# HengyiWang/spann3r

Measured on AMD Instinct MI355X. Metric: frames/sec/GPU (224px, 10-frame seq) + mem-bank cross-attn HBM GB/s, higher is better.
Workload: dtype bf16; 1 GPU; Spann3R.forward, 10-frame 224x224 sequence, batch 1, ViT-L enc / ViT-B dec / DPT heads, eval memory policy; parallelism=sequences sharded 1/GPU x1, hip_graphs=True

## Files before the change

include/spann3r_hip.h:

```cpp
#ifndef SPANN3R_HIP_H
#define SPANN3R_HIP_H

#include <stdint.h>

#ifdef __cplusplus
extern "C" {
#endif

enum { SP3_F32 = 0, SP3_BF16 = 1 };
enum { SP3_ATTN_F32X3 = 2, SP3_ATTN_F16X3 = 3 };
enum { SP3_ACT_NONE = 0, SP3_ACT_GELU = 1, SP3_ACT_RELU = 2 };
enum { SP3_EPI_PLAIN = 0, SP3_EPI_ROPE_VT = 1, SP3_EPI_PIXSHUF = 2, SP3_EPI_PARTIAL = 3 };
enum { SP3_LOAD_PLAIN = 0, SP3_LOAD_CONV3X3 = 1, SP3_LOAD_SOFTMAX = 2 };

const char* sp3_last_error(void);
int sp3_version(void);

int sp3_weight_stream_set(int mode);
int sp3_weight_stream_get(void);

typedef struct sp3_gemm_desc {
  const float* A;
  const float* A2;
  const void* W;
// ... 75 lines not shown
  const float* g2; const float* b2; void* out2; int64_t ld2; int32_t out2_bf16;
  float eps;
  int32_t splits, rows, C;
  int32_t out1_packed, out2_packed;
  int32_t act;
  const float* res2;
  int64_t ldres2;
} sp3_reduce_ln_desc;
int sp3_reduce_ln(const sp3_reduce_ln_desc* desc_host, void* stream);

int sp3_rope_2d(void* tokens, int dtype, int B, int N, int H, int D, int64_t sB, int64_t sN, int64_t sH,
                const int64_t* positions, float base, float fwd, void* stream);

int sp3_attention(const void* q, int64_t sq, int64_t ldq, const void* k, int64_t sk, int64_t ldk,
                  const void* vt, int64_t vt_ld, void* out, int64_t ldo, int out_bf16,
                  int B, int heads, int Nq, int Nk, float scale, int dtype, void* stream);
int sp3_attention_ex(const void* q, int64_t sq, int64_t ldq, const void* k, int64_t sk, int64_t ldk,
                     const void* vt, int64_t vt_ld, void* out, int64_t ldo, int out_bf16, int out_packed,
                     int B, int heads, int Nq, int Nk, float scale, int dtype, void* stream);

int sp3_attention_packed(const void* qp, int q_cols, int q_col0, int npad_q, const void* kp, int k_cols, int k_col0, int npad_k,
                         const void* vtp, void* out, int64_t ldo, int out_bf16, int out_packed,
                         int B, int heads, int Nq, int Nk, float scale, int o_group, int o_group_rows, void* stream);

typedef struct sp3_attn_qproj_desc {
  const void* x_packed; int64_t x_group_stride;
  const float* ln_stats; int64_t stats_group_stride;
  const void* w_packed; int64_t w_group_stride;
  const float* ln_s; const float* bias; int64_t vec_group_stride;
  const int32_t* pos; const float* rope_cos; const float* rope_sin;
  float ln_eps; int32_t D;
  const void* kp; int32_t k_cols, k_col0, npad_k; const void* vtp;
  void* out; int64_t ldo; int32_t out_bf16, out_packed;
  int32_t B, heads, Nq, Nk; float scale; int32_t o_group, o_group_rows;
} sp3_attn_qproj_desc;
int sp3_attention_packed_qproj(const sp3_attn_qproj_desc* desc_host, void* stream);

typedef struct sp3_bank_write_desc {
  const float* feat_k;
  const float* feat_v;
  float* k_raw;
  float* v_raw;
  void* k_hat;
  void* v_hat_t;
  float* s_bank;
  float* b_bank;
  const float *gamma_k, *beta_k, *gamma_v, *beta_v, *gamma_q, *beta_q;
  float eps;
  float alpha;
  int32_t M, P, C, cap;
  int32_t wdtype;
  const int32_t* state;
} sp3_bank_write_desc;
int sp3_bank_write(const sp3_bank_write_desc* desc_host, void* stream);
int sp3_softmax_thresh(const float* S, float* P, int64_t ld, int64_t strideS, int rows, int M, int Mpad,
                       float thresh, int batch, void* P_packed, int64_t stride_packed, int packed_bf16, void* stream);
int sp3_softmax_pack(const float* S, int64_t ld, int64_t strideS, int rows, int M, float thresh, int batch, void* P_packed,
                     int64_t stride_packed, int packed_bf16, float* rowstat_ws, void* stream);
int sp3_colsum_accum(const float* P, int64_t ld, int rows, int M, float* mem_attn, void* stream);
int sp3_colsum_packed(const void* P_packed, int packed_bf16, int rows, int M, float* mem_attn, void* stream);
int sp3_colsum_softmax(const float* S, int64_t ld, int rows, int M, const float* rowz, float thresh, float* mem_attn,
                       float* mem_count, int append_P, void* stream);
int sp3_pack_stats(const float* x, int64_t ldx, int rows, int C, void* packed, int packed_bf16, float* stats, void* stream);
int sp3_gather_packed_rows(const void* src, void* dst, const int32_t* sel, int n_sel, int C, int elem_size, void* stream);
int sp3_gather_packed_cols(const void* src, void* dst, const int32_t* sel, int n_sel, int n_fill, int C, int cap,
                           int elem_size, void* stream);
int sp3_cos_sim(const float* k, const float* wm, int T, int P, int C, float* scratch, float* score, void* stream);
int sp3_bank_state_set(int32_t* state, int M, int wm, void* stream);
int sp3_prob_merge(const float* stats, float* scale, int rows, int M, int cap, const int32_t* dyn_n, void* stream);
int sp3_colsum_prob(const void* P_packed, const float* scale, int rows, int M, int cap, const int32_t* dyn_n, float* mem_attn, void* stream);
int sp3_cos_sim_state(const float* k, const float* k_raw, int Tmax, int P, int C, const int32_t* state, float* scratch, float* score,
                      void* stream);
int sp3_mem_append(float* count, float* attn, int M, int P, void* stream);
int sp3_prune_select(const float* attn, const float* count, int M, float protect, int top_k,
                     int32_t* sel, void* stream);
int sp3_gather_rows(const void* src, void* dst, const int32_t* sel, int n_sel, int C, int elem_size, void* stream);
int sp3_gather_cols(const void* src, int64_t ld_src, void* dst, int64_t ld_dst, const int32_t* sel, int n_sel,
                    int n_fill, int C, int elem_size, void* stream);
int sp3_gather_1d(const float* src, float* dst, const int32_t* sel, int n_sel, void* stream);

int sp3_conv3x3_tile(const void* x, int in_bf16, const void* w_packed, const float* bias, const float* res1,
                     const float* res2, void* out, int out_bf16, int res_bf16, int tile_px, int B, int H, int W,
                     int Cin, int Cout, int relu_in, int act, void* stream);
int sp3_im2col_patch(const float* img, int64_t sb, int64_t sc, int64_t sy, int64_t sx, int B, int C, int H, int W,
                     int p, void* out, int out_bf16, int out_packed, void* stream);
int sp3_upsample2x(const float* in, float* out, int B, int H, int W, int C, int outH, int outW, void* stream);
int sp3_upsample2x_bf16(const void* in, void* out, int B, int H, int W, int C, int outH, int outW, void* stream);
int sp3_head_final(const float* feat, const float* w, const float* b, int64_t pixels, int C, float* pts,
                   float* conf, float* raw, void* stream);
int sp3_head_final_bf16(const void* feat, const float* w, const float* b, int64_t pixels, int C, float* pts, float* conf,
                        float* raw, void* stream);

int sp3_preprocess_image(const uint8_t* src, int64_t src_row_stride, int crop_l, int crop_t, int H1, int W1,
                         const int32_t* hbounds, const int32_t* hcoef, int hksize, int W2,
                         const int32_t* vbounds, const int32_t* vcoef, int vksize, int H2,
                         int crop2_l, int crop2_t, int outW, int outH, int transpose, uint8_t* tmp, float* out, void* stream);

int64_t sp3_conf_loss_ws_bytes(int n, int B);
int sp3_conf_loss_forward(const float* P, const float* Cf, const float* G, const uint8_t* V, const float* pose0, int n, int B, int HW,
                          float alpha, int fix_first, void* ws, float* out7, float* ent_out, void* stream);
int sp3_conf_loss_backward(const float* P, const float* Cf, const float* G, const uint8_t* V, const float* pose0, int n, int B, int HW,
                           float alpha, int fix_first, const void* ws, const float* grad_scale2, float* dP, float* dC, void* stream);
int64_t sp3_ssi_loss_ws_bytes(int n, int B, int HW);
int sp3_ssi_loss_forward(const float* P, const float* G, const uint8_t* V, const float* pose0, int n, int B, int HW, int fix_first,
                         int gt_scale, void* ws, float* out, void* stream);
int sp3_ssi_align_stats(const float* P, const float* G, const uint8_t* V, const float* pose0, int n, int B, int HW, void* ws, float* stats,
                        void* stream);

int sp3_transpose(const float* src, int64_t ld_src, float* dst, int64_t ld_dst, int rows, int cols, void* stream);
int sp3_transpose_batched(const float* src, int64_t ld_src, int64_t stride_src, float* dst, int64_t ld_dst, int64_t stride_dst, int rows,
                          int cols, int batch, void* stream);
int sp3_transpose_pad(const float* src, int64_t ld_src, int64_t stride_src, float* dst, int64_t ld_dst, int64_t stride_dst, int rows,
                      int cols, int batch, int pad_to, void* stream);
int sp3_gelu(const float* x, float* y, int64_t n, void* stream);
int sp3_gelu_bwd(const float* x, const float* dy, float* dx, int64_t n, void* stream);
int sp3_im2col3x3(const float* x, float* col, int B, int H, int W, int C, int stride, void* stream);
int sp3_col2im3x3(const float* dcol, float* dx, int B, int H, int W, int C, int stride, void* stream);
int sp3_relu(const float* x, float* y, int64_t n, void* stream);
int sp3_relu_bwd(const float* x, const float* dy, float* dx, int64_t n, void* stream);
int sp3_upsample2x_bwd(const float* dy, float* dx, int B, int H, int W, int C, int outH, int outW, void* stream);
int sp3_postprocess(const float* raw, float* pts, float* conf, int64_t M, void* stream);
int sp3_postprocess_bwd(const float* raw, const float* dpts, const float* dconf, float* draw, int64_t M, void* stream);
int sp3_adamw(float* p, const float* g, float* m, float* v, int64_t n, float lr, float beta1, float beta2, float eps, float weight_decay,
              int step, float grad_scale, void* stream);
int sp3_mul(const float* a, const float* b, float* out, int64_t n, void* stream);
int sp3_pack_bf16(const float* src, int64_t ld, int rows, int cols, void* dst, void* dstT, void* stream);
int sp3_pack_bf16_conv3x3(const float* x, int B, int H, int W, int C, int stride, int act, void* dst, void* dstT, void* stream);
int sp3_pack_bf16_act(const float* src, int64_t ld, int rows, int cols, void* dst, void* dstT, int act, void* stream);
int sp3_pack_bf16_colsum(const float* src, int64_t ld, int rows, int cols, void* dst, void* dstT, float* colsum, int accumulate,
                         float* partial_ws, void* stream);
int64_t sp3_sumsq_blocks(int64_t n);
int64_t sp3_colsum_rows_ws(int rows, int N);
int sp3_colsum_rows(const float* x, int64_t ld, int rows, int N, float* out, int accumulate, float* scratch, void* stream);
int sp3_sumsq_partial(const float* g, int64_t n, double* partial, void* stream);
int sp3_clip_coef(const double* partial, int count, float max_norm, float extra_scale, float* out, int* step_counter, void* stream);
int sp3_adamw_flat(float* p, const float* g, float* m, float* v, int64_t n, const float* chunk_table, float lr, float beta1, float beta2,
                   float eps, int step, const float* grad_scale_dev, float grad_scale, const int* step_dev, const float* lr_dev, void* stream);
int sp3_softmax_bwd(const float* A, const float* dAd, const float* mask, float* dS, int64_t ld, int rows, int T, float alpha, void* stream);
int sp3_softmax_bwd_pad(const float* A, const float* dAd, const float* mask, float* dS, int64_t ld, int rows, int T, int Tpad, float alpha,
                        void* stream);
typedef struct sp3_head_part {
  const float* src;
  int64_t s_b, s_n, s_h;
  float* dst;
  int64_t d_b, d_n, d_h;
  float* dstT;
  const int64_t* pos;
  int32_t N;
  float fwd;
  int64_t ldT;
} sp3_head_part;
int sp3_head_shuffle(const sp3_head_part* parts, int nparts, int B, int H, int hd, float rope_base, const float* cos_tab,
                     const float* sin_tab, int tab_len, void* stream);
int sp3_attention_train_fwd(const float* q, int64_t sq, int64_t ldq, const float* k, int64_t sk, int64_t ldk, const float* vt, int64_t vt_ld,
                            float* out, int64_t ldo, float* lse, int B, int heads, int Nq, int Nk, float scale, int bf16_products, void* stream);
typedef struct sp3_attn_bwd_desc {
  const float *q, *k, *v, *dout;
  int64_t sq, ldq, sk, ldk, sv, ldv, sdo, lddo;
  const float *qT, *kT, *doT;
  int64_t ldTq, ldTk;
  const float* lse;
  float* D;
  float *dq, *dk, *dv;
  int64_t sdq, lddq, sdk, lddk, sdv, lddv;
  int32_t B, heads, Nq, Nk;
  float scale;
  int32_t bf16_products;
} sp3_attn_bwd_desc;
int sp3_attention_train_bwd(const sp3_attn_bwd_desc* d, void* stream);
int sp3_layernorm_bwd(const float* x, int64_t ldx, const float* gamma, const float* dy, int64_t ldy, const float* dx_add, int64_t ld_add,
                      float* dx, int64_t ld_dx, float* dgamma, float* dbeta, int accumulate, float* scratch, int rows, int C, float eps,
                      void* stream);

int sp3_focal_weiszfeld(const float* pts3d, int B, int H, int W, float ppx, float ppy, int iters, float focal_min, float focal_max,
// ... 184 lines not shown
```

spann3r_amd/csrc/conv.hip:

```cpp
#include "common.h"
#include <type_traits>
#include <cstdlib>

namespace {

constexpr int TH = 8, TW = 8;
constexpr int HP = (TH + 2) * (TW + 2);
constexpr int BM = TH * TW, BN = 64;
constexpr int MF = BM / 16, NF = BN / 16;
constexpr int SLAB_LD = BN + 4;
constexpr int DEPTH = 3;
constexpr int SP3_CONV_WIDE_MIN_WGS = 256;

struct ConvArgs {
  const void* x; const __bf16* w; const float* bias; const float* res1; const float* res2; void* out;
  int B, H, W, Cin, Cout, tiles_x, tiles_y, relu_in, act, out_bf16;
  int xcd_nb;
};

__device__ __forceinline__ bool conv_tile_of(const ConvArgs& a, int& t, int& nblk) {
  t = blockIdx.x; nblk = blockIdx.y;
  if (a.xcd_nb) {
    const unsigned L = blockIdx.x, xc = L & 7, jj = L >> 3, q = jj / (unsigned)a.xcd_nb;
    nblk = (int)(jj - q * a.xcd_nb);
    t = (int)(q * 8 + xc);
    if (t >= a.tiles_x * a.tiles_y * a.B) return false;
  }
  return true;
}

__device__ __forceinline__ bf16x8 ld_frag_lds(const char* p) { return *reinterpret_cast<const bf16x8*>(p); }

template <typename TIN>
__global__ __launch_bounds__(256) void conv3x3_tile_kernel(const ConvArgs a) {
  extern __shared__ __attribute__((aligned(16))) char lds[];
  const int tid = threadIdx.x, lane = tid & 63, wave = tid >> 6, g = lane >> 4, r = lane & 15;
  const int Cin = a.Cin;
  const int PS = Cin * 2 + 16;
  int t, nblk;
  if (!conv_tile_of(a, t, nblk)) return;
  const int tx = t % a.tiles_x; t /= a.tiles_x;
  const int ty = t % a.tiles_y;
  const int b = t / a.tiles_y;
  const int y0 = ty * TH, x0 = tx * TW, n0 = nblk * BN;

  const int upt = Cin >> 5;
  const int U = 9 * upt;
  const int nkb = (9 * Cin) >> 6;
  const __bf16* wb[NF];
#pragma unroll
  for (int n = 0; n < NF; ++n) wb[n] = a.w + ((int64_t)((n0 >> 4) + n) * nkb * 128 + lane) * 8;
  const int nu = (U - wave + 3) >> 2;
  auto w_off = [&](int i) -> int64_t {
    int u = wave + 4 * i;
    u = u < U ? u : U - 1;
    return (int64_t)(u >> 1) * (64 * 16) + (u & 1) * (64 * 8);
  };
  bf16x8 wq[DEPTH][NF];
#pragma unroll
  for (int s = 0; s < DEPTH; ++s) {
    const int64_t o = w_off(s);
#pragma unroll
    for (int n = 0; n < NF; ++n) wq[s][n] = *reinterpret_cast<const bf16x8*>(wb[n] + o);
  }

  {
    constexpr int CHK = 16 / (int)sizeof(TIN);
    const int cpp = Cin / CHK;
    const TIN* xin = reinterpret_cast<const TIN*>(a.x) + (int64_t)b * a.H * a.W * Cin;
    using Chunk = typename std::conditional<sizeof(TIN) == 4, float4, bf16x8>::type;
    auto src_of = [&](int p, int c, bool& ok) -> const Chunk* {
      const int hy = p / (TW + 2), hx = p - hy * (TW + 2);
      const int iy = y0 + hy - 1, ix = x0 + hx - 1;
      ok = p < HP && iy >= 0 && iy < a.H && ix >= 0 && ix < a.W;
      const int cy = ok ? iy : 0, cx = ok ? ix : 0;
      return reinterpret_cast<const Chunk*>(xin + ((int64_t)cy * a.W + cx) * Cin + c);
    };
    auto put = [&](int p, int c, Chunk v, bool ok) {
      char* dst = lds + p * PS + c * 2;
      if constexpr (sizeof(TIN) == 4) {
        if (!ok) v = make_float4(0.f, 0.f, 0.f, 0.f);
        if (a.relu_in) v = relu4(v);
        bf16x4 o;
        o[0] = (__bf16)v.x; o[1] = (__bf16)v.y; o[2] = (__bf16)v.z; o[3] = (__bf16)v.w;
        *reinterpret_cast<bf16x4*>(dst) = o;
      } else {
#pragma unroll
        for (int e = 0; e < 8; ++e) {
          const float f = (float)v[e];
          v[e] = (ok && (!a.relu_in || f > 0.f)) ? v[e] : (__bf16)0.f;
        }
        *reinterpret_cast<bf16x8*>(dst) = v;
      }
    };
    if ((256 % cpp) == 0) {
      const int c = (tid % cpp) * CHK, pstep = 256 / cpp;
      constexpr int NB = 13;
      for (int p0 = tid / cpp; p0 < HP; p0 += NB * pstep) {
        Chunk buf[NB];
        bool ok[NB];
// ... 33 lines not shown
    return (ky * (TW + 2) + kx) * PS + (((c32 >> 1) << 6) + 16 * g + ((c32 & 1) << 3)) * 2;
  };
  bf16x8 af[2][MF];
  {
    const int o = a_off(0);
#pragma unroll
    for (int m = 0; m < MF; ++m) af[0][m] = ld_frag_lds(lds + abase[m] + o);
  }
  for (int i0 = 0; i0 < nu; i0 += 2 * DEPTH) {
#pragma unroll
    for (int s2 = 0; s2 < 2 * DEPTH; ++s2) {
      const int i = i0 + s2;
      if (i < nu) {
        const int s = s2 % DEPTH, cur = s2 & 1;
        {
          const int o = a_off(i + 1);
#pragma unroll
          for (int m = 0; m < MF; ++m) af[cur ^ 1][m] = ld_frag_lds(lds + abase[m] + o);
        }
#pragma unroll
        for (int m = 0; m < MF; ++m)
#pragma unroll
          for (int n = 0; n < NF; ++n)
            acc[m][n] = __builtin_amdgcn_mfma_f32_16x16x32_bf16(af[cur][m], wq[s][n], acc[m][n], 0, 0, 0);
        {
          const int64_t o = w_off(i + DEPTH);
#pragma unroll
          for (int n = 0; n < NF; ++n) wq[s][n] = *reinterpret_cast<const bf16x8*>(wb[n] + o);
        }
      }
    }
  }
  __syncthreads();

  float* slab = reinterpret_cast<float*>(lds) + (size_t)wave * BM * SLAB_LD;
#pragma unroll
  for (int m = 0; m < MF; ++m)
#pragma unroll
    for (int n = 0; n < NF; ++n)
#pragma unroll
      for (int q = 0; q < 4; ++q) slab[(m * 16 + 4 * g + q) * SLAB_LD + n * 16 + r] = acc[m][n][q];
  __syncthreads();
  const float* sm = reinterpret_cast<const float*>(lds);
  for (int idx = tid; idx < BM * (BN / 4); idx += 256) {
    const int row = idx / (BN / 4), c4 = (idx % (BN / 4)) * 4;
    const int oy = y0 + row / TW, ox = x0 + row % TW;
    if (oy >= a.H || ox >= a.W) continue;
    float4 v = *reinterpret_cast<const float4*>(sm + row * SLAB_LD + c4);
#pragma unroll
    for (int s = 1; s < 4; ++s) {
      const float4 t4 = *reinterpret_cast<const float4*>(sm + (size_t)s * BM * SLAB_LD + row * SLAB_LD + c4);
      v.x += t4.x; v.y += t4.y; v.z += t4.z; v.w += t4.w;
    }
    const int gn = n0 + c4;
    if (a.bias) { const float4 b4 = *reinterpret_cast<const float4*>(a.bias + gn); v.x += b4.x; v.y += b4.y; v.z += b4.z; v.w += b4.w; }
    if (a.act == SP3_ACT_RELU) v = relu4(v);
    const int64_t off = (((int64_t)b * a.H + oy) * a.W + ox) * a.Cout + gn;
    if (a.out_bf16 & 2) {
      if (a.res1) { const bf16x4 q = *reinterpret_cast<const bf16x4*>(reinterpret_cast<const __bf16*>(a.res1) + off); v.x += (float)q[0]; v.y += (float)q[1]; v.z += (float)q[2]; v.w += (float)q[3]; }
      if (a.res2) { const bf16x4 q = *reinterpret_cast<const bf16x4*>(reinterpret_cast<const __bf16*>(a.res2) + off); v.x += (float)q[0]; v.y += (float)q[1]; v.z += (float)q[2]; v.w += (float)q[3]; }
    } else {
      if (a.res1) { const float4 q = *reinterpret_cast<const float4*>(a.res1 + off); v.x += q.x; v.y += q.y; v.z += q.z; v.w += q.w; }
      if (a.res2) { const float4 q = *reinterpret_cast<const float4*>(a.res2 + off); v.x += q.x; v.y += q.y; v.z += q.z; v.w += q.w; }
    }
    if (a.out_bf16 & 1) {
      bf16x4 o;
      o[0] = (__bf16)v.x; o[1] = (__bf16)v.y; o[2] = (__bf16)v.z; o[3] = (__bf16)v.w;
      st_out(reinterpret_cast<bf16x4*>(reinterpret_cast<__bf16*>(a.out) + off), o);
    } else {
      st_out(reinterpret_cast<float4*>(reinterpret_cast<float*>(a.out) + off), v);
    }
  }
}

namespace wide {
constexpr int TH = 8, TW = 16, HW = TW + 2, HP = (TH + 2) * HW;
constexpr int CH = 128, PS = CH * 2 + 16;
constexpr int MF = 8;
constexpr int HALO_BYTES = HP * PS;
template <int NF> constexpr int lds_bytes() {
  return HALO_BYTES > 4 * 64 * (16 * NF + 4) * 4 ? HALO_BYTES : 4 * 64 * (16 * NF + 4) * 4;
}

template <typename TIN, int NF = 4, int ABL = 0, bool WS = false>
__global__ __launch_bounds__(256, 2) void conv3x3_wide_kernel(const ConvArgs a) {
  constexpr int BN = 16 * NF, SLAB_LD = BN + 4;
  constexpr int DEPTH = NF == 2 ? 9 : 3;
  static_assert(9 % DEPTH == 0, "the queue slot of a tap must not depend on the chunk");
  extern __shared__ __attribute__((aligned(16))) char lds[];
  const int tid = threadIdx.x, lane = tid & 63, wave = tid >> 6, g = lane >> 4, r = lane & 15;
  const int Cin = a.Cin;
  int t, nblk;
  if (!conv_tile_of(a, t, nblk)) return;
  const int tx = t % a.tiles_x; t /= a.tiles_x;
  const int ty = t % a.tiles_y;
  const int b = t / a.tiles_y;
  const int y0 = ty * TH, x0 = tx * TW, n0 = nblk * BN;
  const int nchunk = Cin / CH, upt = Cin >> 5;
  const int total = 9 * nchunk;

  typedef __attribute__((ext_vector_type(4))) uint32_t u32x4;
  const int nkb = (9 * Cin) >> 6;
  const uint32_t panel_bytes = (uint32_t)nkb * 128 * 8 * 2;
  const auto wrsrc = __builtin_amdgcn_make_buffer_rsrc(
      const_cast<char*>(reinterpret_cast<const char*>(a.w)) + (int64_t)(n0 >> 4) * panel_bytes, 0, (int)(NF * panel_bytes), 0x00020000);
  const uint32_t wlane = (uint32_t)lane * 16 + (uint32_t)(wave & 1) * 1024;
  const int wave_u = __builtin_amdgcn_readfirstlane(wave);
  auto w_off = [&](int c, int tap) -> uint32_t {
    return (uint32_t)((tap * upt + 4 * c + wave_u) >> 1) * 2048;
  };
  auto w_off_seq = [&](int seq) -> uint32_t {
    seq = seq < total ? seq : total - 1;
    const int c = seq / 9;
    return w_off(c, seq - 9 * c);
  };
  auto w_load = [&](uint32_t o, bf16x8* dst) {
#pragma unroll
    for (int n = 0; n < NF; ++n) {
      const u32x4 v = __builtin_amdgcn_raw_buffer_load_b128(wrsrc, wlane, o + n * panel_bytes, WS ? SP3_AUX_STREAM : SP3_AUX_DEFAULT);
      dst[n] = *reinterpret_cast<const bf16x8*>(&v);
    }
  };
  bf16x8 wq[DEPTH][NF];
#pragma unroll
  for (int s = 0; s < DEPTH; ++s) w_load(DEPTH == 9 ? w_off(0, s) : w_off_seq(s), wq[s]);

  f32x4 acc[MF][NF];
#pragma unroll
  for (int m = 0; m < MF; ++m)
#pragma unroll
    for (int n = 0; n < NF; ++n) acc[m][n] = f32x4{0.f, 0.f, 0.f, 0.f};
  const char* abase = lds + r * PS + (((wave >> 1) << 6) + 16 * g + ((wave & 1) << 3)) * 2;

  constexpr int CHK = 16 / (int)sizeof(TIN);
  constexpr int CPP = CH / CHK;
  constexpr int PSTEP = 256 / CPP, NB = sizeof(TIN) == 4 ? 6 : 12;
  const uint32_t img_bytes = (uint32_t)(a.H * a.W * Cin) * (uint32_t)sizeof(TIN);
  const auto rsrc = __builtin_amdgcn_make_buffer_rsrc(
      const_cast<char*>(reinterpret_cast<const char*>(a.x)) + (int64_t)b * img_bytes, 0, (int)img_bytes, 0x00020000);
  const uint32_t xlane = (uint32_t)((tid % CPP) * CHK * sizeof(TIN));
  char* hdst = lds + (tid % CPP) * CHK * 2;

  u32x4 buf[NB];
  auto issue = [&](int c, int p0) {
#pragma unroll
    for (int q = 0; q < NB; ++q) {
      const int p = p0 + q * PSTEP;
      const int hy = p / HW, hx = p - hy * HW;
      const int iy = y0 + hy - 1, ix = x0 + hx - 1;
      const bool ok = p < HP && iy >= 0 && iy < a.H && ix >= 0 && ix < a.W;
      const uint32_t off = ok ? (uint32_t)((iy * a.W + ix) * Cin + c * CH) * (uint32_t)sizeof(TIN) + xlane : 0x80000000u;
      if constexpr (ABL & 4) buf[q] = u32x4{0u, 0u, 0u, 0u};
      else buf[q] = __builtin_amdgcn_raw_buffer_load_b128(rsrc, off, 0, 0);
    }
  };
  auto commit = [&](int p0) {
#pragma unroll
    for (int q = 0; q < NB; ++q) {
      const int p = p0 + q * PSTEP;
      if (p >= HP) continue;
      char* dst = hdst + p * PS;
      if constexpr (sizeof(TIN) == 4) {
        float4 v = make_float4(__uint_as_float(buf[q][0]), __uint_as_float(buf[q][1]), __uint_as_float(buf[q][2]), __uint_as_float(buf[q][3]));
        if (a.relu_in) v = relu4(v);
        bf16x4 o;
        o[0] = (__bf16)v.x; o[1] = (__bf16)v.y; o[2] = (__bf16)v.z; o[3] = (__bf16)v.w;
        *reinterpret_cast<bf16x4*>(dst) = o;
      } else {
        u32x4 v = buf[q];
        if (a.relu_in) {
#pragma unroll
          for (int e = 0; e < 4; ++e) {
            const uint32_t neg = v[e] & 0x80008000u;
            v[e] &= ~((neg >> 15) * 0xffffu);
          }
        }
        *reinterpret_cast<u32x4*>(dst) = v;
      }
    }
  };
  for (int c = 0; c < nchunk; ++c) {
    if (c) __syncthreads();
    for (int p0 = tid / CPP; p0 < HP; p0 += NB * PSTEP) {
      issue(c, p0);
      commit(p0);
    }
    __syncthreads();

    bf16x8 af[MF];
#pragma unroll
    for (int m = 0; m < MF; ++m) af[m] = ld_frag_lds(abase + m * HW * PS);
#pragma unroll
    for (int tap = 0; tap < 9; ++tap) {
      const int s = tap % DEPTH;
      const int nt = tap + 1, nky = nt / 3, nkx = nt - 3 * nky;
#pragma unroll
      for (int m = 0; m < MF; ++m) {
#pragma unroll
        for (int n = 0; n < NF; ++n)
          acc[m][n] = __builtin_amdgcn_mfma_f32_16x16x32_bf16(af[m], wq[s][n], acc[m][n], 0, 0, 0);
        if constexpr (!(ABL & 2))
          if (tap < 8) af[m] = ld_frag_lds(abase + ((m + nky) * HW + nkx) * PS);
      }
      if constexpr (!(ABL & 1)) {
        if constexpr (DEPTH == 9) { if (c + 1 < nchunk) w_load(w_off(c + 1, tap), wq[s]); }
        else w_load(w_off_seq(9 * c + tap + DEPTH), wq[s]);
      }
    }
  }

  float* slab = reinterpret_cast<float*>(lds) + (size_t)wave * 64 * SLAB_LD;
  const float* sm = reinterpret_cast<const float*>(lds);
  if constexpr (ABL & 8) {
    float sum = 0.f;
#pragma unroll
    for (int m = 0; m < MF; ++m)
#pragma unroll
      for (int n = 0; n < NF; ++n) sum += acc[m][n][0] + acc[m][n][1] + acc[m][n][2] + acc[m][n][3];
    if (sum == 12345.678f) reinterpret_cast<float*>(a.out)[tid] = sum;
    return;
  }
#pragma unroll
  for (int h = 0; h < 2; ++h) {
    __syncthreads();
#pragma unroll
    for (int m = 0; m < 4; ++m)
#pragma unroll
      for (int n = 0; n < NF; ++n)
#pragma unroll
        for (int q = 0; q < 4; ++q) slab[(m * 16 + 4 * g + q) * SLAB_LD + n * 16 + r] = acc[4 * h + m][n][q];
    __syncthreads();
    for (int idx = tid; idx < 64 * (BN / 4); idx += 256) {
      const int row = idx / (BN / 4), c4 = (idx % (BN / 4)) * 4;
      const int oy = y0 + 4 * h + (row >> 4), ox = x0 + (row & 15);
      if (oy >= a.H || ox >= a.W) continue;
      float4 v = *reinterpret_cast<const float4*>(sm + row * SLAB_LD + c4);
#pragma unroll
      for (int s = 1; s < 4; ++s) {
        const float4 t4 = *reinterpret_cast<const float4*>(sm + (size_t)s * 64 * SLAB_LD + row * SLAB_LD + c4);
        v.x += t4.x; v.y += t4.y; v.z += t4.z; v.w += t4.w;
      }
      const int gn = n0 + c4;
      if (a.bias) { const float4 b4 = *reinterpret_cast<const float4*>(a.bias + gn); v.x += b4.x; v.y += b4.y; v.z += b4.z; v.w += b4.w; }
      if (a.act == SP3_ACT_RELU) v = relu4(v);
      const int64_t off = (((int64_t)b * a.H + oy) * a.W + ox) * a.Cout + gn;
      if (a.out_bf16 & 2) {
        if (a.res1) { const bf16x4 q = *reinterpret_cast<const bf16x4*>(reinterpret_cast<const __bf16*>(a.res1) + off); v.x += (float)q[0]; v.y += (float)q[1]; v.z += (float)q[2]; v.w += (float)q[3]; }
        if (a.res2) { const bf16x4 q = *reinterpret_cast<const bf16x4*>(reinterpret_cast<const __bf16*>(a.res2) + off); v.x += (float)q[0]; v.y += (float)q[1]; v.z += (float)q[2]; v.w += (float)q[3]; }
      } else {
        if (a.res1) { const float4 q = *reinterpret_cast<const float4*>(a.res1 + off); v.x += q.x; v.y += q.y; v.z += q.z; v.w += q.w; }
        if (a.res2) { const float4 q = *reinterpret_cast<const float4*>(a.res2 + off); v.x += q.x; v.y += q.y; v.z += q.z; v.w += q.w; }
      }
      if (a.out_bf16 & 1) {
        bf16x4 o;
        o[0] = (__bf16)v.x; o[1] = (__bf16)v.y; o[2] = (__bf16)v.z; o[3] = (__bf16)v.w;
        st_out(reinterpret_cast<bf16x4*>(reinterpret_cast<__bf16*>(a.out) + off), o);
      } else {
        st_out(reinterpret_cast<float4*>(reinterpret_cast<float*>(a.out) + off), v);
      }
    }
  }
}

template <typename TIN, int NF, bool WS>
int launch(dim3 grid, hipStream_t st, const ConvArgs& a) {
  constexpr int lds = lds_bytes<NF>();
  auto kern = conv3x3_wide_kernel<TIN, NF, 0, WS>;
  if (lds > 64 * 1024) {
    static bool raised = false;
    if (!raised) {
      hipError_t e = hipFuncSetAttribute(reinterpret_cast<const void*>(kern), hipFuncAttributeMaxDynamicSharedMemorySize, lds);
      if (e != hipSuccess) { sp3_set_error("sp3_conv3x3_tile: cannot raise dynamic LDS to %d: %s", lds, hipGetErrorString(e)); return 2; }
      raised = true;
    }
  }
  hipLaunchKernelGGL(kern, grid, dim3(256), lds, st, a);
  return 0;
}
}

}

extern "C" int sp3_conv3x3_tile(const void* x, int in_bf16, const void* w_packed, const float* bias, const float* res1,
                                const float* res2, void* out, int out_bf16, int res_bf16, int tile_px, int B, int H, int W,
                                int Cin, int Cout, int relu_in, int act, void* stream) {
  SP3_CHECK(x && w_packed && out, "sp3_conv3x3_tile: null pointer");
  SP3_CHECK(B > 0 && H > 0 && W > 0, "sp3_conv3x3_tile: bad shape");
  SP3_CHECK(Cin % 64 == 0 && Cin >= 64 && Cout % 64 == 0 && Cout >= 64, "sp3_conv3x3_tile: Cin=%d / Cout=%d must be multiples of 64", Cin, Cout);
  SP3_CHECK(act == SP3_ACT_NONE || act == SP3_ACT_RELU, "sp3_conv3x3_tile: act %d", act);
  SP3_CHECK(out_bf16 == 0 || out_bf16 == 1, "sp3_conv3x3_tile: out_bf16 %d is not 0 or 1", out_bf16);
  SP3_CHECK(res_bf16 == 0 || res_bf16 == 1, "sp3_conv3x3_tile: res_bf16 %d is not 0 or 1", res_bf16);
  SP3_CHECK(tile_px >= 0 && tile_px <= 3, "sp3_conv3x3_tile: tile_px %d is not 0..3", tile_px);
  auto al16 = [](const void* q) { return (reinterpret_cast<uintptr_t>(q) & 15) == 0; };
  SP3_CHECK(al16(x) && al16(w_packed) && al16(bias) && al16(res1) && al16(res2) && al16(out), "sp3_conv3x3_tile: 16-byte alignment");
  ConvArgs a;
  a.x = x; a.w = reinterpret_cast<const __bf16*>(w_packed); a.bias = bias; a.res1 = res1; a.res2 = res2; a.out = out;
  a.B = B; a.H = H; a.W = W; a.Cin = Cin; a.Cout = Cout;
  a.relu_in = relu_in; a.act = act; a.out_bf16 = out_bf16 | (res_bf16 << 1);
  a.xcd_nb = 0;
  constexpr bool xcd_on = true;
  hipStream_t st = reinterpret_cast<hipStream_t>(stream);
  {
    const int want = tile_px;
    const int wtx = (W + wide::TW - 1) / wide::TW, wty = (H + wide::TH - 1) / wide::TH;
    const int64_t wgs = (int64_t)wtx * wty * B * (Cout / 64);
    const bool can = Cin % wide::CH == 0;
    SP3_CHECK(want < 2 || can, "sp3_conv3x3_tile: the 8 x 16 tile needs Cin %% 128 == 0 (Cin=%d)", Cin);
    SP3_CHECK((int64_t)H * W * Cin * (in_bf16 ? 2 : 4) < (1ll << 31), "sp3_conv3x3_tile: one image of the map must stay below 2 GiB");
    const int nf = want == 2 ? 4 : want == 3 ? 2 : (want == 0 && can) ? (wgs >= SP3_CONV_WIDE_MIN_WGS ? 4 : wgs >= 80 ? 2 : 0) : 0;
    if (nf) {
      a.tiles_x = wtx; a.tiles_y = wty;
      dim3 grid(wtx * wty * B, Cout / (16 * nf));
      if (xcd_on) { a.xcd_nb = Cout / (16 * nf); grid = dim3((unsigned)(((wtx * wty * B + 7) / 8) * 8 * a.xcd_nb), 1); }
      const bool ws = sp3_weight_streams(SP3_WF_CONV_WIDE, nf);
      int rc;
      if (nf == 4) rc = in_bf16 ? (ws ? wide::launch<__bf16, 4, true>(grid, st, a) : wide::launch<__bf16, 4, false>(grid, st, a))
                                : (ws ? wide::launch<float, 4, true>(grid, st, a) : wide::launch<float, 4, false>(grid, st, a));
      else         rc = in_bf16 ? (ws ? wide::launch<__bf16, 2, true>(grid, st, a) : wide::launch<__bf16, 2, false>(grid, st, a))
                                : (ws ? wide::launch<float, 2, true>(grid, st, a) : wide::launch<float, 2, false>(grid, st, a));
      if (rc) return rc;
      SP3_LAUNCH_CHECK("sp3_conv3x3_tile");
      return 0;
    }
  }
  a.tiles_x = (W + TW - 1) / TW; a.tiles_y = (H + TH - 1) / TH;
  const size_t halo = (size_t)HP * (Cin * 2 + 16), slabs = (size_t)4 * BM * SLAB_LD * sizeof(float);
  const size_t lds = halo > slabs ? halo : slabs;
  SP3_CHECK(lds <= 160 * 1024, "sp3_conv3x3_tile: Cin=%d needs %zu bytes of LDS", Cin, lds);
  dim3 grid(a.tiles_x * a.tiles_y * B, Cout / BN);
  if (xcd_on) { a.xcd_nb = Cout / BN; grid = dim3((unsigned)(((a.tiles_x * a.tiles_y * B + 7) / 8) * 8 * a.xcd_nb), 1); }
  auto launch = [&](auto kern) -> int {
    static size_t raised = 0;
    if (lds > 64 * 1024 && lds > raised) {
      raised = lds;
      hipError_t e = hipFuncSetAttribute(reinterpret_cast<const void*>(kern), hipFuncAttributeMaxDynamicSharedMemorySize, (int)lds);
      if (e != hipSuccess) { sp3_set_error("sp3_conv3x3_tile: cannot raise dynamic LDS to %zu: %s", lds, hipGetErrorString(e)); return 2; }
    }
    hipLaunchKernelGGL(kern, grid, dim3(256), lds, st, a);
    return 0;
  };
  const int rc = in_bf16 ? launch(conv3x3_tile_kernel<__bf16>) : launch(conv3x3_tile_kernel<float>);
  if (rc) return rc;
  SP3_LAUNCH_CHECK("sp3_conv3x3_tile");
  return 0;
}
```

spann3r_amd/csrc/dpt.hip:

```cpp
#include "common.h"
#include <math.h>

namespace {

__global__ __launch_bounds__(256) void im2col_patch_kernel(const float* __restrict__ img, int64_t sb, int64_t sc, int64_t sy,
                                                           int64_t sx, int C, int H, int W, int p, void* __restrict__ out,
                                                           int out_bf16, int out_packed, int64_t total) {
  const int64_t idx = (int64_t)blockIdx.x * 256 + threadIdx.x;
  if (idx >= total) return;
  const int K = C * p * p;
  const int64_t row = idx / K;
  const int k = (int)(idx - row * K);
  const int nw = W / p, nh = H / p;
  const int b = (int)(row / (nh * nw));
  const int rem = (int)(row - (int64_t)b * nh * nw);
  const int ty = rem / nw, tx = rem - ty * nw;
  const int c = k / (p * p), r2 = k - c * p * p;
  const int iy = r2 / p, ix = r2 - iy * p;
  const float val = img[b * sb + c * sc + (int64_t)(ty * p + iy) * sy + (int64_t)(tx * p + ix) * sx];
  const int64_t o = out_packed ? packed_off((int)row, k, K, out_bf16 != 0) : idx;
  if (out_bf16) reinterpret_cast<__bf16*>(out)[o] = (__bf16)val;
  else reinterpret_cast<float*>(out)[o] = val;
}

__device__ __forceinline__ float4 ld4(const float* p) { return *reinterpret_cast<const float4*>(p); }
__device__ __forceinline__ float4 ld4(const __bf16* p) {
  const bf16x4 t = *reinterpret_cast<const bf16x4*>(p);
  return make_float4((float)t[0], (float)t[1], (float)t[2], (float)t[3]);
}
__device__ __forceinline__ void st4(float* p, const float4 v) { st_out(reinterpret_cast<float4*>(p), v); }
__device__ __forceinline__ void st4(__bf16* p, const float4 v) {
  bf16x4 t;
  t[0] = (__bf16)v.x; t[1] = (__bf16)v.y; t[2] = (__bf16)v.z; t[3] = (__bf16)v.w;
  st_out(reinterpret_cast<bf16x4*>(p), t);
}

template <typename T>
__global__ __launch_bounds__(256) void upsample2x_kernel(const T* __restrict__ in, T* __restrict__ out, int H, int W,
                                                         int C, int outH, int outW, int64_t total4) {
  const int64_t idx = (int64_t)blockIdx.x * 256 + threadIdx.x;
  if (idx >= total4) return;
  const int c4 = C >> 2;
  const int cc = (int)(idx % c4);
  int64_t pix = idx / c4;
  const int ox = (int)(pix % outW);
  pix /= outW;
  const int oy = (int)(pix % outH);
  const int b = (int)(pix / outH);
  const int OH = 2 * H, OW = 2 * W;
  const float sh = OH > 1 ? (float)(H - 1) / (float)(OH - 1) : 0.f;
  const float sw = OW > 1 ? (float)(W - 1) / (float)(OW - 1) : 0.f;
  const float fy = sh * (float)oy, fx = sw * (float)ox;
  int y0 = (int)fy, x0 = (int)fx;
  y0 = y0 < H - 1 ? y0 : H - 1;
  x0 = x0 < W - 1 ? x0 : W - 1;
  const int y1 = y0 < H - 1 ? y0 + 1 : y0, x1 = x0 < W - 1 ? x0 + 1 : x0;
  const float ly = fy - (float)y0, lx = fx - (float)x0;
  const float hy = 1.f - ly, hx = 1.f - lx;
  const T* base = in + (int64_t)b * H * W * C;
  const float4 v00 = ld4(base + (((int64_t)y0 * W + x0) * c4 + cc) * 4);
  const float4 v01 = ld4(base + (((int64_t)y0 * W + x1) * c4 + cc) * 4);
  const float4 v10 = ld4(base + (((int64_t)y1 * W + x0) * c4 + cc) * 4);
  const float4 v11 = ld4(base + (((int64_t)y1 * W + x1) * c4 + cc) * 4);
  float4 o;
  o.x = hy * (hx * v00.x + lx * v01.x) + ly * (hx * v10.x + lx * v11.x);
  o.y = hy * (hx * v00.y + lx * v01.y) + ly * (hx * v10.y + lx * v11.y);
  o.z = hy * (hx * v00.z + lx * v01.z) + ly * (hx * v10.z + lx * v11.z);
  o.w = hy * (hx * v00.w + lx * v01.w) + ly * (hx * v10.w + lx * v11.w);
  st4(out + idx * 4, o);
}

__global__ __launch_bounds__(256) void upsample2x_bf16x8_kernel(const __bf16* __restrict__ in, __bf16* __restrict__ out, int H, int W,
                                                                int C, int outH, int outW) {
  const int c8 = C >> 3;
  const int t = blockIdx.x * 256 + threadIdx.x;
  if (t >= outW * c8) return;
  const int ox = t / c8, cg = t - ox * c8;
  const int oy = blockIdx.y, b = blockIdx.z;
  const int OH = 2 * H, OW = 2 * W;
  const float sh = OH > 1 ? (float)(H - 1) / (float)(OH - 1) : 0.f;
  const float sw = OW > 1 ? (float)(W - 1) / (float)(OW - 1) : 0.f;
  const float fy = sh * (float)oy, fx = sw * (float)ox;
  int y0 = (int)fy, x0 = (int)fx;
  y0 = y0 < H - 1 ? y0 : H - 1;
  x0 = x0 < W - 1 ? x0 : W - 1;
  const int y1 = y0 < H - 1 ? y0 + 1 : y0, x1 = x0 < W - 1 ? x0 + 1 : x0;
  const float ly = fy - (float)y0, lx = fx - (float)x0;
  const float hy = 1.f - ly, hx = 1.f - lx;
  const __bf16* base = in + (int64_t)b * H * W * C + cg * 8;
  const bf16x8 v00 = *reinterpret_cast<const bf16x8*>(base + ((int64_t)y0 * W + x0) * C);
  const bf16x8 v01 = *reinterpret_cast<const bf16x8*>(base + ((int64_t)y0 * W + x1) * C);
  const bf16x8 v10 = *reinterpret_cast<const bf16x8*>(base + ((int64_t)y1 * W + x0) * C);
  const bf16x8 v11 = *reinterpret_cast<const bf16x8*>(base + ((int64_t)y1 * W + x1) * C);
  bf16x8 o;
#pragma unroll
  for (int e = 0; e < 8; ++e)
    o[e] = (__bf16)(hy * (hx * (float)v00[e] + lx * (float)v01[e]) + ly * (hx * (float)v10[e] + lx * (float)v11[e]));
  st_out(reinterpret_cast<bf16x8*>(out + (((int64_t)b * outH + oy) * outW + ox) * C + cg * 8), o);
}

template <typename T>
__global__ __launch_bounds__(256) void head_final_kernel(const T* __restrict__ feat, const float* __restrict__ w,
                                                         const float* __restrict__ bias, int64_t pixels, int C,
                                                         float* __restrict__ pts, float* __restrict__ conf,
                                                         float* __restrict__ raw) {
  const int64_t gid = (int64_t)blockIdx.x * 256 + threadIdx.x;
  const int64_t pix = gid >> 3;
  const int sub = (int)(gid & 7);
  const bool valid = pix < pixels;
  const int64_t pp = valid ? pix : pixels - 1;
  float a0 = 0.f, a1 = 0.f, a2 = 0.f, a3 = 0.f;
  const T* f = feat + pp * C;
  for (int c = sub * 4; c < C; c += 32) {
    const float4 x = ld4(f + c);
    const float4 w0 = *reinterpret_cast<const float4*>(w + c);
    const float4 w1 = *reinterpret_cast<const float4*>(w + C + c);
    const float4 w2 = *reinterpret_cast<const float4*>(w + 2 * C + c);
    const float4 w3 = *reinterpret_cast<const float4*>(w + 3 * C + c);
    a0 += (x.x * w0.x + x.y * w0.y) + (x.z * w0.z + x.w * w0.w);
    a1 += (x.x * w1.x + x.y * w1.y) + (x.z * w1.z + x.w * w1.w);
    a2 += (x.x * w2.x + x.y * w2.y) + (x.z * w2.z + x.w * w2.w);
    a3 += (x.x * w3.x + x.y * w3.y) + (x.z * w3.z + x.w * w3.w);
  }
#pragma unroll
  for (int o = 1; o < 8; o <<= 1) {
    a0 += __shfl_xor(a0, o); a1 += __shfl_xor(a1, o); a2 += __shfl_xor(a2, o); a3 += __shfl_xor(a3, o);
  }
  if (valid && sub == 0) {
    const float x = a0 + bias[0], y = a1 + bias[1], z = a2 + bias[2], c = a3 + bias[3];
    if (raw) { raw[pix * 4 + 0] = x; raw[pix * 4 + 1] = y; raw[pix * 4 + 2] = z; raw[pix * 4 + 3] = c; }
    const float d = sqrtf(x * x + y * y + z * z);
    const float sc = expm1f(d) / fmaxf(d, 1e-8f);
    pts[pix * 3 + 0] = x * sc; pts[pix * 3 + 1] = y * sc; pts[pix * 3 + 2] = z * sc;
    conf[pix] = 1.0f + expf(c);
  }
}

template <int LP, int PPT>
__global__ __launch_bounds__(256) void head_final_bf16x8_kernel(const __bf16* __restrict__ feat, const float* __restrict__ w,
                                                                const float* __restrict__ bias, int64_t pixels, float* __restrict__ pts,
                                                                float* __restrict__ conf, float* __restrict__ raw) {
  constexpr int C = 8 * LP, PPB = 256 / LP;
  const int li = threadIdx.x % LP, pl = threadIdx.x / LP;
  float wr[4][8];
#pragma unroll
  for (int f = 0; f < 4; ++f) {
    const float4 a = *reinterpret_cast<const float4*>(w + f * C + li * 8), b = *reinterpret_cast<const float4*>(w + f * C + li * 8 + 4);
    wr[f][0] = a.x; wr[f][1] = a.y; wr[f][2] = a.z; wr[f][3] = a.w; wr[f][4] = b.x; wr[f][5] = b.y; wr[f][6] = b.z; wr[f][7] = b.w;
  }
  const float b0 = bias[0], b1 = bias[1], b2 = bias[2], b3 = bias[3];
  const int64_t p0 = (int64_t)blockIdx.x * PPB * PPT + pl;
  bf16x8 x[PPT];
#pragma unroll
  for (int q = 0; q < PPT; ++q) {
    int64_t pix = p0 + (int64_t)q * PPB;
    pix = pix < pixels ? pix : pixels - 1;
    x[q] = *reinterpret_cast<const bf16x8*>(feat + pix * C + li * 8);
  }
#pragma unroll
  for (int q = 0; q < PPT; ++q) {
    const int64_t pix = p0 + (int64_t)q * PPB;
    float a[4];
#pragma unroll
    for (int f = 0; f < 4; ++f) {
      float t0 = 0.f, t1 = 0.f;
#pragma unroll
      for (int e = 0; e < 4; ++e) { t0 = fmaf((float)x[q][e], wr[f][e], t0); t1 = fmaf((float)x[q][4 + e], wr[f][4 + e], t1); }
      a[f] = t0 + t1;
    }
#pragma unroll
    for (int o = 1; o < LP; o <<= 1) {
      a[0] += __shfl_xor(a[0], o); a[1] += __shfl_xor(a[1], o); a[2] += __shfl_xor(a[2], o); a[3] += __shfl_xor(a[3], o);
    }
    if (li == 0 && pix < pixels) {
      const float X = a[0] + b0, Y = a[1] + b1, Z = a[2] + b2, Cc = a[3] + b3;
      if (raw) *reinterpret_cast<float4*>(raw + pix * 4) = make_float4(X, Y, Z, Cc);
      const float d = sqrtf(X * X + Y * Y + Z * Z);
      const float sc = expm1f(d) / fmaxf(d, 1e-8f);
      pts[pix * 3 + 0] = X * sc; pts[pix * 3 + 1] = Y * sc; pts[pix * 3 + 2] = Z * sc;
      conf[pix] = 1.0f + expf(Cc);
    }
  }
}

}

#define ST(s) reinterpret_cast<hipStream_t>(s)

extern "C" int sp3_im2col_patch(const float* img, int64_t sb, int64_t sc, int64_t sy, int64_t sx, int B, int C, int H, int W,
                                int p, void* out, int out_bf16, int out_packed, void* stream) {
  SP3_CHECK(img && out && B > 0 && C > 0 && p > 0, "sp3_im2col_patch: bad arguments");
  SP3_CHECK(H % p == 0 && W % p == 0, "Input image size (%d,%d) is not a multiple of patch size (%d)", H, W, p);
  const int64_t total = (int64_t)B * (H / p) * (W / p) * C * p * p;
  hipLaunchKernelGGL(im2col_patch_kernel, dim3((unsigned)((total + 255) / 256)), dim3(256), 0, ST(stream), img, sb, sc, sy, sx,
                     C, H, W, p, out, out_bf16, out_packed, total);
  SP3_LAUNCH_CHECK("sp3_im2col_patch");
  return 0;
}

extern "C" int sp3_upsample2x(const float* in, float* out, int B, int H, int W, int C, int outH, int outW, void* stream) {
  SP3_CHECK(in && out && B > 0 && H > 0 && W > 0 && C > 0 && C % 4 == 0, "sp3_upsample2x: bad arguments");
  SP3_CHECK(outH > 0 && outH <= 2 * H && outW > 0 && outW <= 2 * W, "sp3_upsample2x: bad crop");
  const int64_t total4 = (int64_t)B * outH * outW * (C / 4);
  hipLaunchKernelGGL(upsample2x_kernel<float>, dim3((unsigned)((total4 + 255) / 256)), dim3(256), 0, ST(stream), in, out, H, W, C,
                     outH, outW, total4);
  SP3_LAUNCH_CHECK("sp3_upsample2x");
  return 0;
}

extern "C" int sp3_upsample2x_bf16(const void* in, void* out, int B, int H, int W, int C, int outH, int outW, void* stream) {
  SP3_CHECK(in && out && B > 0 && H > 0 && W > 0 && C > 0 && C % 4 == 0, "sp3_upsample2x_bf16: bad arguments");
  SP3_CHECK(outH > 0 && outH <= 2 * H && outW > 0 && outW <= 2 * W, "sp3_upsample2x_bf16: bad crop");
  if (C % 8 == 0 && outH <= 65535 && B <= 65535) {
    hipLaunchKernelGGL(upsample2x_bf16x8_kernel, dim3((unsigned)((outW * (C / 8) + 255) / 256), outH, B), dim3(256), 0, ST(stream),
                       reinterpret_cast<const __bf16*>(in), reinterpret_cast<__bf16*>(out), H, W, C, outH, outW);
    SP3_LAUNCH_CHECK("sp3_upsample2x_bf16");
    return 0;
  }
  const int64_t total4 = (int64_t)B * outH * outW * (C / 4);
  hipLaunchKernelGGL(upsample2x_kernel<__bf16>, dim3((unsigned)((total4 + 255) / 256)), dim3(256), 0, ST(stream),
                     reinterpret_cast<const __bf16*>(in), reinterpret_cast<__bf16*>(out), H, W, C, outH, outW, total4);
  SP3_LAUNCH_CHECK("sp3_upsample2x_bf16");
  return 0;
}

extern "C" int sp3_head_final(const float* feat, const float* w, const float* b, int64_t pixels, int C, float* pts, float* conf,
                              float* raw, void* stream) {
  SP3_CHECK(feat && w && b && pts && conf && pixels > 0 && C > 0 && C % 32 == 0, "sp3_head_final: bad arguments");
  const int64_t threads = pixels * 8;
  hipLaunchKernelGGL(head_final_kernel<float>, dim3((unsigned)((threads + 255) / 256)), dim3(256), 0, ST(stream), feat, w, b, pixels, C,
                     pts, conf, raw);
  SP3_LAUNCH_CHECK("sp3_head_final");
  return 0;
}

extern "C" int sp3_head_final_bf16(const void* feat, const float* w, const float* b, int64_t pixels, int C, float* pts, float* conf,
                                   float* raw, void* stream) {
  SP3_CHECK(feat && w && b && pts && conf && pixels > 0 && C > 0 && C % 32 == 0, "sp3_head_final_bf16: bad arguments");
  if (C == 128 && (reinterpret_cast<uintptr_t>(feat) & 15) == 0 && (reinterpret_cast<uintptr_t>(w) & 15) == 0 && (!raw || (reinterpret_cast<uintptr_t>(raw) & 15) == 0)) {
    constexpr int LP = 16, PPT = 4, PPB = 256 / LP;
    hipLaunchKernelGGL((head_final_bf16x8_kernel<LP, PPT>), dim3((unsigned)((pixels + PPB * PPT - 1) / (PPB * PPT))), dim3(256), 0, ST(stream),
                       reinterpret_cast<const __bf16*>(feat), w, b, pixels, pts, conf, raw);
    SP3_LAUNCH_CHECK("sp3_head_final_bf16");
    return 0;
  }
  const int64_t threads = pixels * 8;
  hipLaunchKernelGGL(head_final_kernel<__bf16>, dim3((unsigned)((threads + 255) / 256)), dim3(256), 0, ST(stream),
                     reinterpret_cast<const __bf16*>(feat), w, b, pixels, C, pts, conf, raw);
  SP3_LAUNCH_CHECK("sp3_head_final_bf16");
  return 0;
}
```

spann3r_amd/engine.py:

```python
import math
import os

import torch

from . import ops
from .lib import ACT_NONE, ACT_GELU, ACT_RELU
from .config import Spann3RConfig


def _rope_tables(max_pos, base, device):
    half = 32
    inv_freq = 1.0 / (base ** (torch.arange(0, half, 2).float() / half))
    t = torch.arange(max_pos, dtype=torch.float32)
    ang = torch.einsum("i,j->ij", t, inv_freq)
    return ang.cos().contiguous().to(device), ang.sin().contiguous().to(device)


def _rope_tables_narrow(max_pos, base, head_dim, device):
    D = head_dim // 2
    nf = D // 2
    assert nf <= 16 and head_dim % 4 == 0
    inv_freq = 1.0 / (base ** (torch.arange(0, D, 2).float() / D))
    t = torch.arange(max_pos, dtype=torch.float32)
    ang = torch.einsum("i,j->ij", t, inv_freq)
# ... 480 lines not shown
                                 ln=ops.LnFold(stq, D, w[g + "cq.s"], 1e-6, sb_stats=sb_st, sb_s=D * 4),
                                 strideA=xq.stride, strideW=w[g + "cq.w"].stride, strideC=B * npad * D, sb={"bias": D * 4}, **rope)
                ops.attention_packed(cqp, D, 0, npad, ckp, D, 0, npad, cvtp, ao, D, B=2 * B, heads=Hh, Nq=P, Nk=P,
                                     scale=64 ** -0.5, o_group=B, o_group_rows=Rp)
            upd(ao, D, "cproj", xo, stq, xq)
            Hd = D * cfg.mlp_ratio
            ops.gemm(xq, w[g + "fc1.w"], h, M=R, N=Hd, K=D, lda=D, ldc=Hd, bias=w[g + "fc1.b"], act=ACT_GELU,
                     ln=ops.LnFold(stq, D, w[g + "fc1.s"], 1e-6, sb_stats=sb_st, sb_s=Hd * 4),
                     batch=2, strideA=xq.stride, strideW=w[g + "fc1.w"].stride, strideC=h.stride, sb={"bias": Hd * 4})
            if last:
                upd(h, Hd, "fc2", xo, None, None)
            else:
                upd(h, Hd, "fc2", xo, st[nx], xp[nx])
        normed = self.ws("decg_normed", (2, R, D))
        ops.layernorm(x[depth], w["dec_norm.w"], w["dec_norm.b"], 1e-6, normed, rows=2 * R, C_=D,
                      dual=self.wspg("decg_normed_packed", R, D) if self.adt == torch.bfloat16 else None, group_rows=R)
        outs = {}
        for s_ in (0, 1):
            outs[s_] = [(f1, f2)[s_]] + [x[l][s_].view(B, P, D) for l in range(1, depth)] + [normed[s_].view(B, P, D)]
        return outs[0], outs[1]

    def key_aux(self, R):
        E = self.cfg.enc_dim
        return self.wspg("keyg_packed", R, E), self.ws("keyg_stats", (2, R, E // 32, 2))

    def encode_feat_keys_grouped(self, feat1, feat2, normed1, normed2, R, out1, out2, feat1p=None, feat2p=None, aux=None):
        self.activate()
        cfg, w = self.cfg, self.w
        E, D, Kd = cfg.enc_dim, cfg.dec_dim, cfg.key_dim
        dF, dN, dO = feat2.data_ptr() - feat1.data_ptr(), normed2.data_ptr() - normed1.data_ptr(), out2.data_ptr() - out1.data_ptr()
        assert dF % 16 == 0 and dN % 16 == 0 and dO % 16 == 0
        es = 2 if self.adt == torch.bfloat16 else 4
        h = self.wspg("keyg_hidden", R, Kd)
        packed = None
        if feat1p is not None and feat2p is not None and self.adt == torch.bfloat16 and ops.LEAN:
            np_ = self.wspg("decg_normed_packed", R, D)
            dFp = feat2p.data_ptr() - feat1p.data_ptr()
            assert dFp % 16 == 0
            packed = dict(A2=np_, lda2=D, K1=E, batch=2, strideA=dFp // 2, strideW=w["keyg.0.w"].stride, strideC=h.stride,
                          sb={"bias": Kd * 4, "A2": np_.stride * 2})
            ok = self._splitA_plan.get(R)
            if ok is None:
                ok = self._splitA_plan[R] = ops.gemm(feat1p, w["keyg.0.w"], h, M=R, N=Kd, K=Kd, lda=E, ldc=Kd, bias=w["keyg.0.b"],
                                                     act=ACT_GELU, plan_only=True, **packed) >= 30
            if not ok:
                packed = None
        if packed is not None:
            ops.gemm(feat1p, w["keyg.0.w"], h, M=R, N=Kd, K=Kd, lda=E, ldc=Kd, bias=w["keyg.0.b"], act=ACT_GELU, **packed)
        else:
            ops.gemm(feat1, w["keyg.0.w"], h, M=R, N=Kd, K=Kd, lda=E, ldc=Kd, bias=w["keyg.0.b"], act=ACT_GELU, A2=normed1, lda2=D, K1=E,
                     batch=2, strideA=dF // 4, strideW=w["keyg.0.w"].stride, strideC=h.stride, sb={"bias": Kd * 4, "A2": dN})
        kp, kst = aux or self.key_aux(R)
        ops.gemm(h, w["keyg.2.w"], out1, M=R, N=E, K=Kd, lda=Kd, ldc=E, bias=w["keyg.2.b"], stats_out=kst, c2=kp,
                 batch=2, strideA=h.stride, strideW=w["keyg.2.w"].stride, strideC=dO // 4,
                 sb={"bias": E * 4, "stats_out": R * (E // 32) * 8, "c2": kp.stride * es})
        return kp.at(1), kst[1]

    def encode_feat_key(self, feat, dec_last, R, num, out, aux=False):
        self.activate()
        cfg, w = self.cfg, self.w
        E, D, Kd = cfg.enc_dim, cfg.dec_dim, cfg.key_dim
        h = self.wsp("key_hidden%d" % num, R, Kd)
        pre = "key%d." % num
        ops.gemm(feat, w[pre + "0.w"], h, M=R, N=Kd, K=Kd, lda=E, ldc=Kd, bias=w[pre + "0.b"], act=ACT_GELU,
                 A2=dec_last, lda2=D, K1=E)
        if aux:
            kp, kst = self.key_aux(R) if aux is True else aux
            ops.gemm(h, w[pre + "2.w"], out, M=R, N=E, K=Kd, lda=Kd, ldc=E, bias=w[pre + "2.b"], stats_out=kst[num - 1],
                     c2=kp.at(num - 1))
            return kp.at(num - 1), kst[num - 1]
        ops.gemm(h, w[pre + "2.w"], out, M=R, N=E, K=Kd, lda=Kd, ldc=E, bias=w[pre + "2.b"])
        return out

    def _conv_ws(self, head):
        return self.ws("conv_splitk_ws" + str(head), (1 << 23,))

    def _rcu_c1(self, x, pre, B, H, W_, tag=""):
        w, F = self.w, self.cfg.dpt_feat
        t = self.ws("rcu_tmp" + tag, (B * H * W_, F), self.mdt)
        ops.conv3x3(x, w[pre + "c1.w"], t, B=B, H=H, W_=W_, Cin=F, Cout=F, bias=w[pre + "c1.b"], relu_in=True, act=ACT_RELU,
                    splitk_ws=self._conv_ws(tag[:1]))
        return t

    def _rcu(self, x, pre, B, H, W_, out, extra_res=None, tag="", c1_done=False, extra_up=None):
        w, F = self.w, self.cfg.dpt_feat
        t = self.ws("rcu_tmp" + tag, (B * H * W_, F), self.mdt)
        if not c1_done:
            self._rcu_c1(x, pre, B, H, W_, tag)
        ops.conv3x3(t, w[pre + "c2.w"], out, B=B, H=H, W_=W_, Cin=F, Cout=F, bias=w[pre + "c2.b"], res1=x, res2=extra_res,
                    splitk_ws=self._conv_ws(tag[:1]), res2_up=extra_up)
        return out

    def _fusion(self, pre, B, H, W_, x0, x1, tag, crop=None, c1_done=False, x0_up=None, fold_up=False):
        w, F = self.w, self.cfg.dpt_feat
        M = B * H * W_
        cur = x0
        if x1 is not None:
            s = self.ws("fus_sum_" + tag, (M, F), self.mdt)
            self._rcu(x1, pre + "u1", B, H, W_, s, extra_res=x0, tag=tag, c1_done=c1_done, extra_up=x0_up)
            cur = s
        r = self.ws("fus_rcu2_" + tag, (M, F), self.mdt)
        self._rcu(cur, pre + "u2", B, H, W_, r, tag=tag, c1_done=c1_done and x1 is None)
        oc = self.ws("fus_oc_" + tag, (M, F), self.mdt)
        ops.gemm(r, w[pre + "out.w"], oc, M=M, N=F, K=F, lda=F, ldc=F, bias=w[pre + "out.b"])
        OH, OW = (2 * H, 2 * W_) if crop is None else crop
        if fold_up:
            return oc, OH, OW
        up = self.ws("fus_up_" + tag, (B * OH * OW, F), self.mdt)
        ops.upsample2x(oc, up, B=B, H=H, W_=W_, C_=F, outH=OH, outW=OW)
        return up, OH, OW

    def dpt_head(self, dec, B, nh, nw, num, want_raw=False):
        self.activate()
        cfg, w = self.cfg, self.w
        F, Lc = cfg.dpt_feat, cfg.dpt_last
        pre = "dpt%d." % num
        R = B * nh * nw
        hk = cfg.hooks
        dims = (cfg.enc_dim, cfg.dec_dim, cfg.dec_dim, cfg.dec_dim)
        ld = (96, 192, 384, 768)
        mdt = self.mdt
        t = [self.ws("dpt%d_pp%d" % (num, i), (R, ld[i]), mdt) for i in range(4)]
        import contextlib
        lv = ops.HEAD_LEVELS
        group = ops.level if len({dec[hk[i]].dtype for i in range(4)}) == 1 else contextlib.nullcontext
        with (group if lv else contextlib.nullcontext)():
            for i0 in (0, 2):
                with (contextlib.nullcontext if lv else group)():
                    for i in (i0, i0 + 1):
                        ops.gemm(dec[hk[i]], w[pre + "pp%d.w" % i], t[i], M=R, N=ld[i], K=dims[i], lda=dims[i], ldc=ld[i], bias=w[pre + "pp%d.b" % i])
        c0 = 128 if self.wdt == torch.bfloat16 else ld[0]
        l0 = self.ws("dpt%d_l0" % num, (B * 16 * nh * nw, c0), mdt)
        l1 = self.ws("dpt%d_l1" % num, (B * 4 * nh * nw, ld[1]), mdt)
        with group():
            ops.conv_transpose_ks(t[0], w[pre + "pp0t.w"], l0, B=B, H=nh, W_=nw, Cin=ld[0], Cout=c0, ks=4, bias=w[pre + "pp0t.b"])
            ops.conv_transpose_ks(t[1], w[pre + "pp1t.w"], l1, B=B, H=nh, W_=nw, Cin=ld[1], Cout=ld[1], ks=2, bias=w[pre + "pp1t.b"])
        l2 = t[2]
        h3, w3 = (nh - 1) // 2 + 1, (nw - 1) // 2 + 1
        l3 = self.ws("dpt%d_l3" % num, (B * h3 * w3, ld[3]), mdt)
        sk = self._conv_ws(num)
        geo = ((4 * nh, 4 * nw), (2 * nh, 2 * nw), (nh, nw), (h3, w3))
        srcs = (l0, l1, l2, l3)
        rn = [self.ws("dpt%d_rn%d" % (num, i), (B * geo[i][0] * geo[i][1], F), mdt) for i in range(4)]

        def layer_rn(i):
            ops.conv3x3(srcs[i], w[pre + "rn%d.w" % i], rn[i], B=B, H=geo[i][0], W_=geo[i][1], Cin=(c0 if i == 0 else ld[i]), Cout=F, splitk_ws=sk)

        def pp3c():
            ops.conv3x3(t[3], w[pre + "pp3c.w"], l3, B=B, H=nh, W_=nw, Cin=ld[3], Cout=ld[3], stride=2, bias=w[pre + "pp3c.b"], splitk_ws=sk)

        refs = [(pre + "ref%d." % (4 - j), "%d_%d" % (num, 4 - j)) for j in range(4)]
        if lv:
            with ops.level():
                pp3c()
                layer_rn(2)
            with ops.level():
                layer_rn(0)
                layer_rn(1)
                layer_rn(3)
                self._rcu_c1(rn[2], refs[1][0] + "u1", B, geo[2][0], geo[2][1], refs[1][1])
            with ops.level():
                self._rcu_c1(rn[3], refs[0][0] + "u2", B, geo[3][0], geo[3][1], refs[0][1])
                self._rcu_c1(rn[1], refs[2][0] + "u1", B, geo[1][0], geo[1][1], refs[2][1])
                self._rcu_c1(rn[0], refs[3][0] + "u1", B, geo[0][0], geo[0][1], refs[3][1])
        else:
            pp3c()
            for i in range(4):
                layer_rn(i)
        path, up, Hc, Wc = rn[3], None, h3, w3
        for j in range(4):
            Hn, Wn = geo[3 - j]
            fold = lv and j < 3 and ops.conv3x3_takes_res2_up(w[refs[j + 1][0] + "u1c2.w"], mdt, B, *geo[2 - j])
            nxt, OH_, OW_ = self._fusion(refs[j][0], B, Hn, Wn, path, rn[3 - j] if j else None, refs[j][1], crop=(nh, nw) if j == 0 else None,
                                         c1_done=lv, x0_up=up, fold_up=fold)
            path, up = nxt, ((Hn, Wn) if fold else None)
        p1, H1, W1 = path, OH_, OW_
        a = self.ws("dpt%d_h0" % num, (B * H1 * W1, Lc), mdt)
        ops.conv3x3(p1, w[pre + "h0.w"], a, B=B, H=H1, W_=W1, Cin=F, Cout=Lc, bias=w[pre + "h0.b"])
        OH, OW = 2 * H1, 2 * W1
        u = self.ws("dpt%d_h0up" % num, (B * OH * OW, Lc), mdt)
        ops.upsample2x(a, u, B=B, H=H1, W_=W1, C_=Lc)
        c = self.ws("dpt%d_h2" % num, (B * OH * OW, Lc), mdt)
        ops.conv3x3(u, w[pre + "h2.w"], c, B=B, H=OH, W_=OW, Cin=Lc, Cout=Lc, bias=w[pre + "h2.b"], act=ACT_RELU)
        pts = self.ws("dpt_pts%d" % num, (B, OH, OW, 3))
        conf = self.ws("dpt_conf%d" % num, (B, OH, OW))
        raw = self.ws("dpt_raw%d" % num, (B, OH, OW, 4)) if want_raw else None
        ops.head_final(c, w[pre + "h4.w"], w[pre + "h4.b"], B * OH * OW, Lc, pts, conf, raw)
        return pts, conf, raw

    def encode_cur_value_feat(self, tok, out, res, pos32=None):
        self.activate()
        cfg, w = self.cfg, self.w
        B, P, Cv = tok.shape
        assert Cv == cfg.val_dim
        R, E = B * P, cfg.enc_dim
        zero_pos = self.ws("valf_zero_pos", (R, 2), torch.int32, zero=True)
        rope_tab = None
        if cfg.mem_pos_enc:
            assert pos32 is not None and self.rope_narrow is not None
            zero_pos, rope_tab = pos32, self.rope_narrow
        x = self.ws("valf_x", (R, Cv))
        xpA, xpB = self.wsp("valf_xpA", R, Cv), self.wsp("valf_xpB", R, Cv)
        stA, stB = self.stats("valf_stA", R, Cv), self.stats("valf_stB", R, Cv)
        ops.copy2d(tok.reshape(R, Cv), Cv, x, Cv, R, Cv)
        ops.pack_stats(x, xpA, stA, rows=R, C_=Cv)
        for i in range(cfg.val_depth):
            self._block(x, xpA, stA, xpB, stB, R, B, P, Cv, cfg.enc_heads, "val%d." % i, zero_pos, tag="_valf",
                        head_dim=Cv // cfg.enc_heads, rope_tab=rope_tab)
        ops.gemm(xpA, w["value_out.w"], out, M=R, N=E, K=Cv, lda=Cv, ldc=E, bias=w["value_out.b"], res1=res, ldr1=E,
                 ln=ops.LnFold(stA, Cv, w["value_out.s"], 1e-6))
        return out

    def encode_cur_value(self, pts3d, out, res):
        self.activate()
        cfg, w = self.cfg, self.w
        B, H, W_, _ = pts3d.shape
        p, E = cfg.patch, cfg.enc_dim
        nh, nw = H // p, W_ // p
        P = nh * nw
        R = B * P
        _, pos32, zero_pos = self.positions(B, nh, nw)
        col = self.wsp("im2col_val", R, 3 * p * p)
        sb, sy, sx, sc = pts3d.stride()
        ops.im2col_patch(pts3d, col, B=B, C_=3, H=H, W_=W_, p=p, strides=(sb, sc, sy, sx))
        x, xp, st = self._vit(col, R, B, P, "pospatch", "val", cfg.val_depth, pos32 if cfg.mem_pos_enc else zero_pos, tag="_val")
        ops.gemm(xp, w["value_out.w"], out, M=R, N=E, K=E, lda=E, ldc=E, bias=w["value_out.b"], res1=res, ldr1=E,
                 ln=ops.LnFold(st, E, w["value_out.s"], 1e-6))
        return out
```

spann3r_amd/lib.py:

```python
import ctypes as C
import os

import torch

_HERE = os.path.dirname(os.path.abspath(__file__))
LIB_PATH = os.environ.get("SP3_LIB_PATH") or os.path.join(_HERE, "libspann3r_hip.so")

F32, BF16 = 0, 1
ATTN_F32X3, ATTN_F16X3 = 2, 3
ACT_NONE, ACT_GELU, ACT_RELU = 0, 1, 2
EPI_PLAIN, EPI_ROPE_VT, EPI_PIXSHUF, EPI_PARTIAL = 0, 1, 2, 3
LOAD_PLAIN, LOAD_CONV3X3, LOAD_SOFTMAX = 0, 1, 2


class GemmDesc(C.Structure):
    _fields_ = [
        ("A", C.c_void_p), ("A2", C.c_void_p), ("W", C.c_void_p), ("C", C.c_void_p), ("bias", C.c_void_p),
        ("res1", C.c_void_p), ("res2", C.c_void_p),
        ("M", C.c_int32), ("N", C.c_int32), ("K", C.c_int32), ("batch", C.c_int32),
        ("K1", C.c_int32),
        ("lda", C.c_int64), ("lda2", C.c_int64), ("ldw", C.c_int64), ("ldc", C.c_int64),
        ("ldr1", C.c_int64), ("ldr2", C.c_int64),
        ("strideA", C.c_int64), ("strideW", C.c_int64), ("strideC", C.c_int64),
        ("alpha", C.c_float), ("wdtype", C.c_int32), ("act", C.c_int32), ("out_bf16", C.c_int32),
# ... 73 lines not shown
    _fields_ = [("ox", C.c_float), ("oy", C.c_float), ("oz", C.c_float), ("h", C.c_float), ("inv_h", C.c_float), ("slack", C.c_float),
                ("nx", C.c_int32), ("ny", C.c_int32), ("nz", C.c_int32)]


class RenderCam(C.Structure):
    _fields_ = [("R", C.c_float * 9), ("t", C.c_float * 3), ("fx", C.c_float), ("fy", C.c_float), ("cx", C.c_float), ("cy", C.c_float),
                ("width", C.c_int32), ("height", C.c_int32), ("z_near", C.c_float), ("point_size", C.c_int32)]


class ViewDesc(C.Structure):
    _fields_ = [("src", C.c_void_p), ("row_stride", C.c_int64), ("dtype", C.c_int32), ("src_w", C.c_int32), ("src_h", C.c_int32),
                ("crop_l", C.c_int32), ("crop_t", C.c_int32), ("W1", C.c_int32), ("H1", C.c_int32), ("W2", C.c_int32), ("H2", C.c_int32),
                ("l2", C.c_int32), ("t2", C.c_int32), ("w", C.c_int32), ("h", C.c_int32), ("transpose", C.c_int32),
                ("fu", C.c_float), ("fv", C.c_float), ("cu", C.c_float), ("cv", C.c_float), ("pose", C.c_float * 12),
                ("use_raw_invalid", C.c_int32), ("raw_invalid", C.c_float), ("depth_div", C.c_float), ("min_depth", C.c_float),
                ("max_depth", C.c_float)]


class TsdfFrame(C.Structure):
    _fields_ = [("depth", C.c_void_p), ("pts", C.c_void_p), ("valid", C.c_void_p), ("pixel_weight", C.c_void_p), ("rgba", C.c_void_p),
                ("row_stride", C.c_int64), ("w", C.c_int32), ("h", C.c_int32), ("fu", C.c_float), ("fv", C.c_float), ("cu", C.c_float),
                ("cv", C.c_float), ("w2c", C.c_float * 12)]


class TsdfView(C.Structure):
    _fields_ = [("depth", C.c_void_p), ("vertex", C.c_void_p), ("normal", C.c_void_p), ("rgba", C.c_void_p), ("row_stride", C.c_int64),
                ("w", C.c_int32), ("h", C.c_int32), ("fu", C.c_float), ("fv", C.c_float), ("cu", C.c_float), ("cv", C.c_float),
                ("c2w", C.c_float * 12), ("near", C.c_float), ("far", C.c_float)]


_lib = None

_PROTOS = {
    "sp3_gemm": [C.POINTER(GemmDesc), C.c_void_p],
    "sp3_gemm_n": [C.POINTER(C.POINTER(GemmDesc)), C.c_int, C.c_void_p],
    "sp3_gemm_plan_n": [C.POINTER(C.POINTER(GemmDesc)), C.c_int, C.POINTER(C.c_int)],
    "sp3_gemm_plan": [C.POINTER(GemmDesc)],
    "sp3_layernorm": [C.c_void_p, C.c_int64, C.c_void_p, C.c_void_p, C.c_float, C.c_void_p, C.c_int64, C.c_int,
                      C.c_int, C.c_int, C.c_void_p],
    "sp3_reduce_ln": [C.POINTER(ReduceLnDesc), C.c_void_p],
    "sp3_layernorm_dual": [C.c_void_p, C.c_int64, C.c_void_p, C.c_void_p, C.c_float, C.c_void_p, C.c_int64, C.c_void_p, C.c_int, C.c_int,
                           C.c_int, C.c_int, C.c_void_p],
    "sp3_layernorm_packed": [C.c_void_p, C.c_int64, C.c_void_p, C.c_void_p, C.c_float, C.c_void_p, C.c_int,
                             C.c_int, C.c_int, C.c_void_p],
    "sp3_attention_ex": [C.c_void_p, C.c_int64, C.c_int64, C.c_void_p, C.c_int64, C.c_int64, C.c_void_p, C.c_int64,
                         C.c_void_p, C.c_int64, C.c_int, C.c_int, C.c_int, C.c_int, C.c_int, C.c_int, C.c_float, C.c_int,
                         C.c_void_p],
    "sp3_layernorm_t": [C.c_void_p, C.c_int64, C.c_void_p, C.c_void_p, C.c_float, C.c_void_p, C.c_int64, C.c_int,
                        C.c_int, C.c_int, C.c_void_p],
    "sp3_rope_2d": [C.c_void_p, C.c_int, C.c_int, C.c_int, C.c_int, C.c_int, C.c_int64, C.c_int64, C.c_int64,
                    C.c_void_p, C.c_float, C.c_float, C.c_void_p],
    "sp3_attention": [C.c_void_p, C.c_int64, C.c_int64, C.c_void_p, C.c_int64, C.c_int64, C.c_void_p, C.c_int64,
                      C.c_void_p, C.c_int64, C.c_int, C.c_int, C.c_int, C.c_int, C.c_int, C.c_float, C.c_int, C.c_void_p],
    "sp3_attention_packed": [C.c_void_p, C.c_int, C.c_int, C.c_int, C.c_void_p, C.c_int, C.c_int, C.c_int, C.c_void_p,
                             C.c_void_p, C.c_int64, C.c_int, C.c_int, C.c_int, C.c_int, C.c_int, C.c_int, C.c_float, C.c_int, C.c_int,
                             C.c_void_p],
    "sp3_attention_packed_qproj": [C.POINTER(AttnQProjDesc), C.c_void_p],
    "sp3_softmax_thresh": [C.c_void_p, C.c_void_p, C.c_int64, C.c_int64, C.c_int, C.c_int, C.c_int, C.c_float,
                           C.c_int, C.c_void_p, C.c_int64, C.c_int, C.c_void_p],
    "sp3_softmax_pack": [C.c_void_p, C.c_int64, C.c_int64, C.c_int, C.c_int, C.c_float, C.c_int, C.c_void_p, C.c_int64, C.c_int, C.c_void_p,
                         C.c_void_p],
    "sp3_colsum_packed": [C.c_void_p, C.c_int, C.c_int, C.c_int, C.c_void_p, C.c_void_p],
    "sp3_colsum_softmax": [C.c_void_p, C.c_int64, C.c_int, C.c_int, C.c_void_p, C.c_float, C.c_void_p, C.c_void_p, C.c_int, C.c_void_p],
    "sp3_bank_write": [C.POINTER(BankWriteDesc), C.c_void_p],
    "sp3_pack_stats": [C.c_void_p, C.c_int64, C.c_int, C.c_int, C.c_void_p, C.c_int, C.c_void_p, C.c_void_p],
    "sp3_gather_packed_rows": [C.c_void_p, C.c_void_p, C.c_void_p, C.c_int, C.c_int, C.c_int, C.c_void_p],
    "sp3_gather_packed_cols": [C.c_void_p, C.c_void_p, C.c_void_p, C.c_int, C.c_int, C.c_int, C.c_int, C.c_int, C.c_void_p],
    "sp3_colsum_accum": [C.c_void_p, C.c_int64, C.c_int, C.c_int, C.c_void_p, C.c_void_p],
    "sp3_cos_sim": [C.c_void_p, C.c_void_p, C.c_int, C.c_int, C.c_int, C.c_void_p, C.c_void_p, C.c_void_p],
    "sp3_mem_append": [C.c_void_p, C.c_void_p, C.c_int, C.c_int, C.c_void_p],
    "sp3_bank_state_set": [C.c_void_p, C.c_int, C.c_int, C.c_void_p],
    "sp3_prob_merge": [C.c_void_p, C.c_void_p, C.c_int, C.c_int, C.c_int, C.c_void_p, C.c_void_p],
    "sp3_colsum_prob": [C.c_void_p, C.c_void_p, C.c_int, C.c_int, C.c_int, C.c_void_p, C.c_void_p, C.c_void_p],
    "sp3_cos_sim_state": [C.c_void_p, C.c_void_p, C.c_int, C.c_int, C.c_int, C.c_void_p, C.c_void_p, C.c_void_p, C.c_void_p],
    "sp3_prune_select": [C.c_void_p, C.c_void_p, C.c_int, C.c_float, C.c_int, C.c_void_p, C.c_void_p],
    "sp3_gather_rows": [C.c_void_p, C.c_void_p, C.c_void_p, C.c_int, C.c_int, C.c_int, C.c_void_p],
    "sp3_gather_cols": [C.c_void_p, C.c_int64, C.c_void_p, C.c_int64, C.c_void_p, C.c_int, C.c_int, C.c_int,
                        C.c_int, C.c_void_p],
    "sp3_gather_1d": [C.c_void_p, C.c_void_p, C.c_void_p, C.c_int, C.c_void_p],
    "sp3_im2col_patch": [C.c_void_p, C.c_int64, C.c_int64, C.c_int64, C.c_int64, C.c_int, C.c_int, C.c_int, C.c_int,
                         C.c_int, C.c_void_p, C.c_int, C.c_int, C.c_void_p],
    "sp3_conv3x3_tile": [C.c_void_p, C.c_int, C.c_void_p, C.c_void_p, C.c_void_p, C.c_void_p, C.c_void_p, C.c_int, C.c_int, C.c_int,
                         C.c_int, C.c_int, C.c_int, C.c_int, C.c_int, C.c_int, C.c_int, C.c_void_p],
    "sp3_upsample2x": [C.c_void_p, C.c_void_p, C.c_int, C.c_int, C.c_int, C.c_int, C.c_int, C.c_int, C.c_void_p],
    "sp3_head_final": [C.c_void_p, C.c_void_p, C.c_void_p, C.c_int64, C.c_int, C.c_void_p, C.c_void_p, C.c_void_p,
                       C.c_void_p],
    "sp3_upsample2x_bf16": [C.c_void_p, C.c_void_p, C.c_int, C.c_int, C.c_int, C.c_int, C.c_int, C.c_int, C.c_void_p],
    "sp3_head_final_bf16": [C.c_void_p, C.c_void_p, C.c_void_p, C.c_int64, C.c_int, C.c_void_p, C.c_void_p, C.c_void_p,
                            C.c_void_p],
    "sp3_fill_f32": [C.c_void_p, C.c_float, C.c_int64, C.c_void_p],
    "sp3_cast_f32_to_bf16": [C.c_void_p, C.c_void_p, C.c_int64, C.c_void_p],
    "sp3_copy2d_f32": [C.c_void_p, C.c_int64, C.c_void_p, C.c_int64, C.c_int, C.c_int, C.c_void_p],
    "sp3_spin": [C.c_int64, C.c_void_p, C.c_void_p],
    "sp3_conf_loss_forward": [C.c_void_p, C.c_void_p, C.c_void_p, C.c_void_p, C.c_void_p, C.c_int, C.c_int, C.c_int, C.c_float, C.c_int,
                              C.c_void_p, C.c_void_p, C.c_void_p, C.c_void_p],
    "sp3_conf_loss_backward": [C.c_void_p, C.c_void_p, C.c_void_p, C.c_void_p, C.c_void_p, C.c_int, C.c_int, C.c_int, C.c_float, C.c_int,
                               C.c_void_p, C.c_void_p, C.c_void_p, C.c_void_p, C.c_void_p],
    "sp3_transpose": [C.c_void_p, C.c_int64, C.c_void_p, C.c_int64, C.c_int, C.c_int, C.c_void_p],
    "sp3_transpose_batched": [C.c_void_p, C.c_int64, C.c_int64, C.c_void_p, C.c_int64, C.c_int64, C.c_int, C.c_int, C.c_int, C.c_void_p],
    "sp3_transpose_pad": [C.c_void_p, C.c_int64, C.c_int64, C.c_void_p, C.c_int64, C.c_int64, C.c_int, C.c_int, C.c_int, C.c_int, C.c_void_p],
    "sp3_softmax_bwd_pad": [C.c_void_p, C.c_void_p, C.c_void_p, C.c_void_p, C.c_int64, C.c_int, C.c_int, C.c_int, C.c_float, C.c_void_p],
    "sp3_head_shuffle": [C.c_void_p, C.c_int, C.c_int, C.c_int, C.c_int, C.c_float, C.c_void_p, C.c_void_p, C.c_int, C.c_void_p],
    "sp3_attention_train_fwd": [C.c_void_p, C.c_int64, C.c_int64, C.c_void_p, C.c_int64, C.c_int64, C.c_void_p, C.c_int64, C.c_void_p, C.c_int64,
                                C.c_void_p, C.c_int, C.c_int, C.c_int, C.c_int, C.c_float, C.c_int, C.c_void_p],
    "sp3_attention_train_bwd": [C.c_void_p, C.c_void_p],
    "sp3_gelu": [C.c_void_p, C.c_void_p, C.c_int64, C.c_void_p],
    "sp3_gelu_bwd": [C.c_void_p, C.c_void_p, C.c_void_p, C.c_int64, C.c_void_p],
    "sp3_im2col3x3": [C.c_void_p, C.c_void_p, C.c_int, C.c_int, C.c_int, C.c_int, C.c_int, C.c_void_p],
    "sp3_col2im3x3": [C.c_void_p, C.c_void_p, C.c_int, C.c_int, C.c_int, C.c_int, C.c_int, C.c_void_p],
    "sp3_relu": [C.c_void_p, C.c_void_p, C.c_int64, C.c_void_p],
    "sp3_relu_bwd": [C.c_void_p, C.c_void_p, C.c_void_p, C.c_int64, C.c_void_p],
    "sp3_upsample2x_bwd": [C.c_void_p, C.c_void_p, C.c_int, C.c_int, C.c_int, C.c_int, C.c_int, C.c_int, C.c_void_p],
    "sp3_postprocess": [C.c_void_p, C.c_void_p, C.c_void_p, C.c_int64, C.c_void_p],
    "sp3_postprocess_bwd": [C.c_void_p, C.c_void_p, C.c_void_p, C.c_void_p, C.c_int64, C.c_void_p],
    "sp3_adamw": [C.c_void_p, C.c_void_p, C.c_void_p, C.c_void_p, C.c_int64, C.c_float, C.c_float, C.c_float, C.c_float, C.c_float, C.c_int,
                  C.c_float, C.c_void_p],
    "sp3_mul": [C.c_void_p, C.c_void_p, C.c_void_p, C.c_int64, C.c_void_p],
    "sp3_pack_bf16": [C.c_void_p, C.c_int64, C.c_int, C.c_int, C.c_void_p, C.c_void_p, C.c_void_p],
    "sp3_pack_bf16_conv3x3": [C.c_void_p, C.c_int, C.c_int, C.c_int, C.c_int, C.c_int, C.c_int, C.c_void_p, C.c_void_p, C.c_void_p],
    "sp3_pack_bf16_act": [C.c_void_p, C.c_int64, C.c_int, C.c_int, C.c_void_p, C.c_void_p, C.c_int, C.c_void_p],
    "sp3_pack_bf16_colsum": [C.c_void_p, C.c_int64, C.c_int, C.c_int, C.c_void_p, C.c_void_p, C.c_void_p, C.c_int, C.c_void_p, C.c_void_p],
    "sp3_colsum_rows": [C.c_void_p, C.c_int64, C.c_int, C.c_int, C.c_void_p, C.c_int, C.c_void_p, C.c_void_p],
    "sp3_sumsq_partial": [C.c_void_p, C.c_int64, C.c_void_p, C.c_void_p],
    "sp3_clip_coef": [C.c_void_p, C.c_int, C.c_float, C.c_float, C.c_void_p, C.c_void_p, C.c_void_p],
    "sp3_adamw_flat": [C.c_void_p, C.c_void_p, C.c_void_p, C.c_void_p, C.c_int64, C.c_void_p, C.c_float, C.c_float, C.c_float, C.c_float,
                       C.c_int, C.c_void_p, C.c_float, C.c_void_p, C.c_void_p, C.c_void_p],
    "sp3_softmax_bwd": [C.c_void_p, C.c_void_p, C.c_void_p, C.c_void_p, C.c_int64, C.c_int, C.c_int, C.c_float, C.c_void_p],
    "sp3_layernorm_bwd": [C.c_void_p, C.c_int64, C.c_void_p, C.c_void_p, C.c_int64, C.c_void_p, C.c_int64, C.c_void_p, C.c_int64,
                          C.c_void_p, C.c_void_p, C.c_int, C.c_void_p, C.c_int, C.c_int, C.c_float, C.c_void_p],
    "sp3_focal_weiszfeld": [C.c_void_p, C.c_int, C.c_int, C.c_int, C.c_float, C.c_float, C.c_int, C.c_float, C.c_float, C.c_void_p, C.c_void_p],
    "sp3_conf_filter": [C.c_void_p, C.c_void_p, C.c_void_p, C.c_int64, C.c_float, C.c_void_p, C.c_void_p, C.c_void_p, C.c_void_p, C.c_void_p],
    "sp3_copy_multi": [C.c_int, C.c_void_p, C.c_void_p, C.c_void_p, C.c_void_p],
    "sp3_pnp_dlt_accum": [C.c_void_p, C.c_int, C.c_int, C.c_int, C.c_float, C.c_float, C.c_float, C.c_void_p, C.c_void_p, C.c_float, C.c_int,
                          C.c_void_p, C.c_void_p],
    "sp3_pnp_gn_accum": [C.c_void_p, C.c_int, C.c_int, C.c_int, C.c_float, C.c_float, C.c_float, C.c_void_p, C.c_void_p, C.c_float, C.c_void_p, C.c_void_p],
    "sp3_pnp_score": [C.c_void_p, C.c_int, C.c_int, C.c_int, C.c_float, C.c_float, C.c_float, C.c_void_p, C.c_int, C.c_float, C.c_int, C.c_void_p, C.c_void_p],
    "sp3_ssi_loss_forward": [C.c_void_p, C.c_void_p, C.c_void_p, C.c_void_p, C.c_int, C.c_int, C.c_int, C.c_int, C.c_int, C.c_void_p, C.c_void_p,
                             C.c_void_p],
    "sp3_preprocess_image": [C.c_void_p, C.c_int64, C.c_int, C.c_int, C.c_int, C.c_int, C.c_void_p, C.c_void_p, C.c_int, C.c_int,
                             C.c_void_p, C.c_void_p, C.c_int, C.c_int, C.c_int, C.c_int, C.c_int, C.c_int, C.c_int, C.c_void_p,
                             C.c_void_p, C.c_void_p],
    "sp3_nn_cell_ids": [C.c_void_p, C.c_int64, C.POINTER(NnGrid), C.c_void_p, C.c_void_p],
    "sp3_nn_pack_records": [C.c_void_p, C.c_void_p, C.c_int64, C.c_void_p, C.c_void_p],
    "sp3_nn_query": [C.c_void_p, C.c_void_p, C.c_int64, C.c_void_p, C.c_void_p, C.c_int64, C.POINTER(NnGrid), C.c_int, C.c_float, C.c_void_p,
                     C.c_void_p, C.c_void_p, C.c_void_p],
    "sp3_nn_brute": [C.c_void_p, C.c_int64, C.c_void_p, C.c_int64, C.c_float, C.c_void_p, C.c_void_p, C.c_void_p, C.c_void_p],
    "sp3_knn_query": [C.c_void_p, C.c_void_p, C.c_int64, C.c_void_p, C.c_void_p, C.c_int64, C.POINTER(NnGrid), C.c_int, C.c_float,
                      C.c_void_p, C.c_void_p, C.c_void_p],
    "sp3_knn_normals": [C.c_void_p, C.c_void_p, C.c_int64, C.c_int, C.c_void_p, C.c_void_p],
    "sp3_transform_points": [C.c_void_p, C.c_int64, C.POINTER(C.c_double), C.c_void_p, C.c_void_p],
    "sp3_icp_accum": [C.c_void_p, C.c_void_p, C.c_void_p, C.c_int64, C.c_void_p, C.c_void_p, C.c_void_p],
    "sp3_sum_count_f32": [C.c_void_p, C.c_int64, C.c_float, C.c_void_p, C.c_void_p, C.c_void_p],
    "sp3_normal_dot": [C.c_void_p, C.c_void_p, C.c_void_p, C.c_int64, C.c_int, C.c_void_p, C.c_void_p],
    "sp3_render_clear": [C.c_void_p, C.c_int64, C.c_void_p],
    "sp3_render_splat": [C.c_void_p, C.c_void_p, C.c_float, C.c_int64, C.c_int64, C.POINTER(RenderCam), C.c_void_p, C.c_void_p],
    "sp3_render_resolve": [C.c_void_p, C.c_void_p, C.POINTER(RenderCam), C.c_uint32, C.c_void_p, C.c_void_p, C.c_void_p, C.c_void_p],
    "sp3_pack_rgba8": [C.c_void_p, C.c_int64, C.c_void_p, C.c_void_p],
    "sp3_colorize_hsv": [C.c_void_p, C.c_int64, C.c_void_p, C.c_void_p],
    "sp3_colorize_lut": [C.c_void_p, C.c_int64, C.c_void_p, C.c_void_p, C.c_void_p],
    "sp3_mesh_faces": [C.c_void_p, C.c_void_p, C.c_float, C.c_void_p, C.c_int, C.c_int, C.c_int, C.c_int, C.c_void_p, C.c_void_p, C.c_void_p,
                       C.c_void_p, C.c_void_p],
    "sp3_mesh_compact_vertices": [C.c_void_p, C.c_void_p, C.c_int64, C.c_void_p, C.c_int64, C.c_void_p, C.c_void_p, C.c_float, C.c_float,
                                  C.POINTER(C.c_float), C.c_void_p, C.c_void_p, C.c_void_p, C.c_void_p, C.c_void_p, C.c_void_p],
    "sp3_mesh_components": [C.c_void_p, C.c_int64, C.c_int64, C.c_void_p, C.c_int64, C.c_void_p, C.c_void_p, C.c_void_p, C.c_void_p, C.c_void_p,
                            C.c_void_p],
    "sp3_mesh_select_faces": [C.c_void_p, C.c_void_p, C.c_int64, C.c_void_p, C.c_int64, C.c_void_p, C.c_void_p, C.c_void_p, C.c_void_p],
    "sp3_mesh_cluster": [C.c_void_p, C.c_void_p, C.c_int64, C.POINTER(C.c_float), C.c_float, C.c_int, C.c_void_p, C.c_void_p, C.c_void_p,
                         C.c_void_p, C.c_void_p, C.c_void_p],
    "sp3_mesh_cluster_faces": [C.c_void_p, C.c_int64, C.c_void_p, C.c_int64, C.c_int, C.c_int, C.c_void_p, C.c_void_p, C.c_void_p, C.c_void_p],
    "sp3_mesh_face_frames": [C.c_void_p, C.c_int64, C.c_void_p, C.c_int64, C.c_void_p, C.c_void_p, C.c_void_p, C.c_void_p, C.c_void_p],
    "sp3_mesh_sample": [C.c_void_p, C.c_void_p, C.c_int64, C.c_void_p, C.c_int64, C.c_void_p, C.c_void_p, C.c_int64, C.c_uint64, C.c_void_p,
                        C.c_void_p, C.c_void_p, C.c_void_p, C.c_void_p],
# ... 109 lines not shown
```

spann3r_amd/model.py:

```python
import argparse
import collections
import os
import weakref

import torch
import torch.nn as nn

from . import ops
from .config import Spann3RConfig, FULL
from .engine import Engine
from .weights import param_spec, alias_of, synth_state_dict


def _build_param_tree(root: nn.Module, spec):
    made = {}
    for key, shape in spec.items():
        parts = key.split(".")
        mod = root
        for name in parts[:-1]:
            if not hasattr(mod, name) or not isinstance(getattr(mod, name), nn.Module):
                mod.add_module(name, nn.Module())
            mod = getattr(mod, name)
        src = alias_of(key)
        if src is not None:
# ... 633 lines not shown
        return outs

    def begin_outputs(self, n_steps):
        self._out_slabs, self._out_steps, self._out_i = None, n_steps, 0

    def _step_outputs(self, srcs):
        if getattr(self, "_out_steps", 0) <= 0 or self._out_i >= self._out_steps:
            return [torch.empty_like(t) for t in srcs]
        if self._out_slabs is None or len(self._out_slabs) != len(srcs):
            self._out_slabs = [t.new_empty((self._out_steps,) + tuple(t.shape)) for t in srcs]
        i, self._out_i = self._out_i, self._out_i + 1
        return [slab[i] for slab in self._out_slabs]

    def pair_copies(self, i):
        B = self.B
        pairs = [(self.feats[i * B:(i + 2) * B], self.featpair)]
        if self.feats_p is not None:
            st = self.feats_p.stride
            pairs.append((self.feats_p.data.view(-1)[i * st:(i + 2) * st], self.featpair_p.data.view(-1)[:2 * st]))
        return pairs

    def load_pair(self, i):
        ops.copy_multi(self.pair_copies(i))

    def _part1(self, first, has_next, scores_to_host, stream=False):
        eng, mem, B, P, E = self.eng, self.mem, self.B, self.P, self.E
        main = torch.cuda.current_stream()
        st = eng.side_streams()
        packed = self.packed_feats and self.model.packed_features and self.batched and self.feats_p is not None
        p1 = p2 = f1p = None
        if packed:
            p1, p2 = self.featpair_p.at(0), self.featpair_p.at(1)
        if first:
            if not self.batched:
                eng.encode_image(self.img_pair, out=self.featpair)
            f1, f1p = self.feat1, p1
        else:
            if stream:
                ops.copy2d(self.feat2, E, self.feat1, E, B * P, E)
                st[3].wait_stream(main)
                with torch.cuda.stream(st[3]):
                    eng.encode_image(self.img_next, out=self.feat2, tag="_pre")
            elif not self.batched:
                ops.copy2d(self.feat2, E, self.feat1, E, B * P, E)
                ops.copy2d(self.feat_pre, E, self.feat2, E, B * P, E)
            mem.memory_read(self.k2, self.fuse, *(self.k2_aux if B == 1 else (None, None)), defer_attn=True,
                            out_packed=self.fuse_p if packed else None)
            f1 = self.fuse
            f1p = self.fuse_p if (packed and mem.wrote_packed) else None
            if stream:
                main.wait_stream(st[3])
        if has_next:
            st[3].wait_stream(main)
            with torch.cuda.stream(st[3]):
                eng.encode_image(self.img_next, out=self.feat_pre, tag="_pre")
        if eng.packed_attn and self.model.grouped_decoder:
            dec1, dec2 = eng.decoder_grouped(f1, self.feat2, B, self.nh, self.nw, f1p=f1p, f2p=p2 if f1p is not None else None)
            self.k2_aux = eng.encode_feat_keys_grouped(self.feat1, self.feat2, dec1[-1], dec2[-1], B * P, self.k1, self.k2,
                                                       feat1p=p1, feat2p=p2, aux=self.own_aux)
        else:
            dec1, dec2 = eng.decoder(f1, self.feat2, B, self.nh, self.nw, self.nh, self.nw, streams=st)
            st[2].wait_stream(main)
            with torch.cuda.stream(st[2]):
                self.k2_aux = eng.encode_feat_key(self.feat2, dec2[-1], B * P, 2, self.k2, aux=self.own_aux or True)
            eng.encode_feat_key(self.feat1, dec1[-1], B * P, 1, self.k1)
            main.wait_stream(st[2])
        if not self.training and mem.sim_needed():
            mem.sim_scores(self.k1, to_host=scores_to_host and mem.state is not None)
        if has_next:
            main.wait_stream(st[3])
        self.dec = (dec1, dec2)
        self.dec2_hooks = [dec2[h] for h in self.model.cfg.hooks[1:]]

    def _part2(self):
        eng, mem, B = self.eng, self.mem, self.B
        dec1, dec2 = self.dec
        main = torch.cuda.current_stream()
        st = eng.side_streams()
        pts2 = conf2 = None
        if not self.defer2:
            st[2].wait_stream(main)
            with torch.cuda.stream(st[2]):
                pts2, conf2, _ = eng.dpt_head(dec2, B, self.hh, self.hw, 2)
        pts1, conf1, _ = eng.dpt_head(dec1, B, self.hh, self.hw, 1)
        if eng.cfg.use_feat:
            eng.encode_cur_value_feat(dec1[-1], self.v, self.k1,
                                      pos32=eng.positions(B, self.nh, self.nw)[1] if eng.cfg.mem_pos_enc else None)
        else:
            eng.encode_cur_value(pts1.swapaxes(1, 2) if self.swap else pts1, self.v, self.k1)
        mem.stage_write(self.k1, self.v)
        if not self.defer2:
            main.wait_stream(st[2])
        self.out = (pts1, conf1, pts2, conf2)

    def run(self, first, has_next, use_graphs, post_copies=(), stream=False):
        mem = self.mem
        has_next = has_next and not self.batched
        gk = mem.graph_key()
        per_length = 0 if gk[0] in ("s", "p") else 1 if (stream or mem.state is not None) else self._out_steps
        if not use_graphs and ops._prof is not None:
            ops._prof.step_begin()
        need_sim = not self.training and mem.sim_needed()
        if need_sim:
            mem.arm_score_poll()

        def whole():
            self._part1(first, has_next, need_sim, stream)
            if need_sim and mem.state is None:
                mem.copy_scores_to_host()
            self._part2()
        key = ("whole", first, need_sim) + gk + (has_next, self.batched, self.defer2, self.model.grouped_decoder, self.model.packed_features,
                                                 stream)
        self.graphs.run(key, whole, use_graphs and ops._prof is None, per_length)
        if not first:
            mem.note_deferred_read()
        pts1, conf1, pts2, conf2 = self.out
        srcs = (pts1, conf1) + (() if pts2 is None else (pts2, conf2))
        outs = self._step_outputs(srcs)
        copies = list(zip(srcs, outs))
        copies += list(post_copies() if callable(post_copies) else post_copies)
        for c0 in range(0, len(copies), 8):
            ops.copy_multi(copies[c0:c0 + 8])
        res1 = {"pts3d": outs[0], "conf": outs[1]}
        res2 = {} if pts2 is None else {"pts3d": outs[2], "conf": outs[3]}
        if self.swap:
            res1 = {k: v.swapaxes(1, 2) for k, v in res1.items()}
            res2 = {k: v.swapaxes(1, 2) for k, v in res2.items()}
        if self.training:
            mem.commit_staged()
        else:
            mem.finish_staged(mem.sim_verdict() if need_sim else False)
        return res1, res2


class Spann3R(nn.Module):

    def __init__(self, dus3r_name="./checkpoints/DUSt3R_ViTLarge_BaseDecoder_512_dpt.pth",
                 use_feat=False, mem_pos_enc=False, memory_dropout=0.15, cfg: Spann3RConfig = None,
                 init_weights=True):
        super().__init__()
        self.use_feat = use_feat
        self.mem_pos_enc = mem_pos_enc
        self.mem_dropout = nn.Dropout(memory_dropout)
        ckpt = None
        if dus3r_name is not None and not os.path.isfile(dus3r_name):
            raise FileNotFoundError("DUSt3R checkpoint %r not found (pass dus3r_name=None to build without one)" % dus3r_name)
        if dus3r_name is not None:
            torch.serialization.add_safe_globals([argparse.Namespace])
            ckpt = torch.load(dus3r_name, map_location="cpu", weights_only=True)
            cfg = Spann3RConfig.from_ctor_string(ckpt["args"].model)
        self.cfg = cfg or FULL
        if mem_pos_enc != self.cfg.mem_pos_enc or use_feat != self.cfg.use_feat:
            import dataclasses
            self.cfg = dataclasses.replace(self.cfg, mem_pos_enc=bool(mem_pos_enc), use_feat=bool(use_feat))
        self.add_module("dust3r", _Dust3RFacade(self))
        self._params = _build_param_tree(self, param_spec(self.cfg))
        if init_weights:
            with torch.no_grad():
                for k, v in synth_state_dict(0, self.cfg).items():
                    if alias_of(k) is None:
                        self._params[k].copy_(v)
        if ckpt is not None:
            sd = {("dust3r." + k): v for k, v in ckpt["model"].items()}
            if not any(k.startswith("dust3r.dec_blocks2") for k in sd):
                for k, v in list(sd.items()):
                    if k.startswith("dust3r.dec_blocks."):
                        sd[k.replace("dust3r.dec_blocks.", "dust3r.dec_blocks2.")] = v
            own = self.state_dict()
            missing = [k for k in own if k.startswith("dust3r.") and k not in sd and alias_of(k) is None]
            unexpected = [k for k in sd if k not in own]
            print("<checkpoint %s: missing keys %s, unexpected keys %s>" % (dus3r_name, missing, unexpected))
            with torch.no_grad():
# ... 405 lines not shown
```

spann3r_amd/ops.py:

```python
import ctypes as C

import torch

from . import lib as L
from .lib import GemmDesc, F32, BF16, ATTN_F32X3, ATTN_F16X3, ACT_NONE, ACT_GELU, ACT_RELU


_prof = None


class Profiler:

    def __init__(self, blocker_ms=12.0):
        self.rec = []
        self.regions = []
        self.blocker_cycles = int(blocker_ms * 2.4e6)

    def step_begin(self):
        torch.cuda._sleep(self.blocker_cycles)

    def region_begin(self):
        return (self.begin(), len(self.rec))

    def region_end(self, key, e0, nbytes, info=None):
        e1 = torch.cuda.Event(enable_timing=True)
        e1.record()
        e0, n0 = e0
        self.regions.append((key, e0, e1, float(nbytes), info, len(self.rec) - n0))

    def region_summary(self):
        torch.cuda.synchronize()
        ov = getattr(self, "bracket_ms", 0.0)
        out = []
        for k, e0, e1, b, i, inner in self.regions:
            raw = e0.elapsed_time(e1)
            out.append(dict(key=k, ms=max(raw - ov * (inner + 1), 1e-4), raw_ms=raw, launches=inner, bytes=b, info=i))
        return out

    def begin(self):
        e = torch.cuda.Event(enable_timing=True)
        e.record()
        return e

    def end(self, key, e0, flops, nbytes):
        e1 = torch.cuda.Event(enable_timing=True)
        e1.record()
        self.rec.append((key, e0, e1, float(flops), float(nbytes)))

    def calibrate(self, n=40):
        ticks = torch.zeros(n, dtype=torch.int64, device="cuda")
        torch.cuda.synchronize()
        self.step_begin()
        ev = []
        for i in range(n):
            e0 = torch.cuda.Event(enable_timing=True)
            e1 = torch.cuda.Event(enable_timing=True)
            e0.record()
            L.check(L.load().sp3_spin(12000, ticks[i:].data_ptr(), L.stream_ptr()), "sp3_spin")
            e1.record()
            ev.append((e0, e1))
        torch.cuda.synchronize()
        dur_ms = (ticks.cpu().double() * 1e-5).tolist()
        t = sorted(a.elapsed_time(b) - d for (a, b), d in zip(ev, dur_ms))
        self.bracket_ms = max(t[len(t) // 2], 0.0)
        return self.bracket_ms

    def summary(self):
        torch.cuda.synchronize()
        agg = {}
        ov = getattr(self, "bracket_ms", 0.0)
        for key, e0, e1, fl, by in self.rec:
            a = agg.setdefault(key, dict(launches=0, ms=0.0, flops=0.0, bytes=0.0))
            a["launches"] += 1
            a["ms"] += max(e0.elapsed_time(e1) - ov, 1e-4)
            a["flops"] += fl
            a["bytes"] += by
        return agg


def set_profiler(p):
    global _prof
    _prof = p


_TILE_NAMES = {0: "32x32xk4", 1: "64x64", 2: "64x128", 3: "64x64xk4", 5: "128x128lds", 6: "128x64lds", 13: "112x64wreg8",
               20: "256x128pipe", 21: "128x128pipe", 22: "128x64pipe", 24: "64x32pipe", 25: "32x32pipe",
               30: "lean-rope-k1024-48x64xk8", 31: "lean-rope-k768-32x32xk4", 32: "lean-packed-k1024-64x64xk8", 33: "lean-packed-k768-32x32xk4",
               34: "lean-stream-k1024-32x32xk8", 35: "lean-stream-k4096-32x32xk8r4", 36: "lean-stream-k768-48x32xk6",
               37: "lean-stream-k3072-48x32xk8", 38: "lean-stream-k1792-64x32xk7",
               39: "lean-stream-k1024-48x32xk8", 40: "lean-conv-16x16xk12", 41: "lean-conv-32x32xk8", 42: "lean-packed-splitA-k1792-64x32xk7", 43: "lean-score-k1024-32x32xk8", 44: "lean-softmax-pv-16x64xk8",
               45: "lean-prob-k1024-256x128", 46: "lean-prob-pv-256x128",
               50: "lean-rope-k1024-256x128", 51: "lean-rope-k1024-128x128", 52: "lean-rope-k768-128x128", 53: "lean-packed-k1024-256x128",
               54: "lean-packed-k1024-128x128", 55: "lean-packed-k768-128x128", 56: "lean-stream-k1024-128x64", 57: "lean-stream-k4096-128x64",
               58: "lean-stream-k768-128x64", 59: "lean-stream-k3072-128x64", 60: "lean-stream-k1792-128x64",
               61: "lean-stream-k1024-256x128", 62: "lean-stream-k4096-256x128", 63: "lean-rope-k768-256x128", 64: "lean-packed-k768-256x128", 65: "lean-rope-k768-128x64", 66: "lean-packed-splitA-k1792-128x128", 67: "lean-packed-splitA-k1792-256x128"}


import os as _os
import threading as _threading
PROF_SHAPES = _os.environ.get("SP3_PROF_SHAPES", "0")[:1] == "1"
LEAN = _os.environ.get("SP3_LEAN_GEMM", "1")[:1] != "0"

HEAD_LEVELS = _os.environ.get("SP3_HEAD_LEVELS", "1")[:1] != "0"
_held = None


def level_block_map(problems):
    start = [0]
    for tile, M, N in problems:
        bm = 16 if tile == 40 else 32
        start.append(start[-1] + 8 * ((M + bm - 1) // bm) * ((N // bm + 7) // 8))

    def f(w):
        p = max(i for i in range(len(problems)) if w >= start[i])
        tile, M, N = problems[p]
        bm = 16 if tile == 40 else 32
        mt = (M + bm - 1) // bm
        local = w - start[p]
        j = local >> 3
        return p, j % mt, (j // mt) * 8 + (local & 7)
    return start[-1], f


def level_order(problems):
    cost = [(K // 64) * (2 if tile == 40 else 3) for tile, K in problems]
    return sorted(range(len(problems)), key=lambda i: -cost[i])


class level:

    def __enter__(self):
        global _held
        assert _held is None
        _held = []
        return self

    def __exit__(self, et, ev, tb):
        global _held
        held, _held = _held, None
        if et is not None:
            return False
        conv = [x[0].loader == L.LOAD_CONV3X3 for x in held]
        if any(conv) and not all(conv):
            raise RuntimeError("ops.level(): small-map convolutions and other GEMMs do not share a launch")
        for i in range(0, len(held), 4):
            self._send(held[i:i + 4], any(conv))
        return False

    @staticmethod
    def _send(group, is_conv):
        if len(group) == 1:
            _gemm_launch(group[0][0], "sp3_gemm", group[0][1])
            return
        ds = [g[0] for g in group]
        arr = (C.POINTER(GemmDesc) * len(ds))(*[C.pointer(d) for d in ds])
        e0 = _prof.begin() if _prof is not None else None
        L.check(L.load().sp3_gemm_n(arr, len(ds), L.stream_ptr()), "sp3_gemm_n")
        if _prof is not None:
            tiles = (C.c_int * len(ds))()
            L.check(L.load().sp3_gemm_plan_n(arr, len(ds), tiles), "sp3_gemm_plan_n")
            cost = [_gemm_cost(d) for d in ds]
            a = ds[0]
            head = "<A%s,W%s,%s," % ("bf16" if a.a_bf16 else "f32", "f32" if a.wdtype == F32 else "bf16", group[0][1])
            if len(ds) == 2 and not is_conv:
                key = "gemm2" + head + _TILE_NAMES[tiles[0]] + ">"
            else:
                key = "gemm_n" + head + "+".join(sorted({_TILE_NAMES[t] for t in tiles})) + " x%d>" % len(ds)
            _prof.end(key, e0, sum(c[0] for c in cost), sum(c[1] for c in cost))


pair = level


def _gemm_cost(d):
    b = max(d.batch, 1)
    wsz = 4 if d.wdtype == F32 else 2
    asz, csz = (2 if d.a_bf16 else 4), (2 if d.out_bf16 else 4)
    a_elems = d.M * d.K if d.loader != L.LOAD_CONV3X3 else d.M * d.conv_stride * d.conv_stride * d.conv_C
    return 2.0 * d.M * d.N * d.K * b, b * (asz * a_elems + wsz * d.N * d.K + csz * d.M * d.N)


def _gemm_launch(d, what, loader_name):
    if _held is not None:
        _held.append((d, loader_name))
        return
    if _prof is None:
# ... 160 lines not shown
    d.batch, d.strideA, d.strideW, d.strideC = batch, strideA, strideW, strideC
    for k, v in (sb or {}).items():
        setattr(d, "sb_" + k, v)


def wdtype_of(t):
    if t.dtype == torch.float32:
        return F32
    if t.dtype == torch.bfloat16:
        return BF16
    raise TypeError("weights must be float32 or bfloat16, got %s" % t.dtype)


def _f32(t, name):
    if t is not None and (t.dtype != torch.float32 or not t.is_cuda):
        raise TypeError("%s must be a float32 CUDA(HIP) tensor" % name)


def _is_packed(t):
    return int(isinstance(t, PackedAct))


def _act(t, name):
    if not t.is_cuda or t.dtype not in (torch.float32, torch.bfloat16):
        raise TypeError("%s must be a float32/bfloat16 CUDA(HIP) tensor" % name)
    return int(t.dtype == torch.bfloat16)


def gemm(A, W, out, *, M, N, K, lda, ldc, bias=None, res1=None, ldr1=0, res2=None, ldr2=0, act=ACT_NONE, alpha=1.0,
         relu_in=False, tile=-1, batch=1, strideA=0, strideW=0, strideC=0, ldw=0,
         A2=None, lda2=0, K1=0, splitk=0, ln=None, stats_out=None, c2=None, sb=None, trace=None,
         sm_stats_out=None, softmax=None, plan_only=False, dyn_n=None):
    d = GemmDesc()
    d.a_bf16 = _act(A, "A")
    d.a_packed = _is_packed(A)
    d.out_packed = _is_packed(out)
    out_bf16 = out.dtype == torch.bfloat16
    _w(d, W)
    d.A, d.A2, d.C = A.data_ptr(), L.ptr(A2), out.data_ptr()
    d.bias, d.res1, d.res2 = L.ptr(bias), L.ptr(res1), L.ptr(res2)
    d.M, d.N, d.K, d.batch, d.K1 = M, N, K, batch, K1
    d.lda, d.lda2, d.ldw, d.ldc, d.ldr1, d.ldr2 = lda, lda2, ldw, ldc, ldr1, ldr2
    d.strideA, d.strideW, d.strideC = strideA, strideW, strideC
    d.alpha, d.act, d.out_bf16, d.relu_in = alpha, act, int(out_bf16), int(relu_in)
    d.loader, d.epi, d.tile = L.LOAD_PLAIN, L.EPI_PLAIN, tile
    if splitk >= 1:
        d.epi, d.splitk = L.EPI_PARTIAL, splitk
    _ln(d, ln)
    d.stats_out, d.c2 = L.ptr(stats_out), L.ptr(c2)
    d.trace = L.ptr(trace)
    d.sm_stats_out = L.ptr(sm_stats_out)
    d.dyn_n = L.ptr(dyn_n)
    if softmax is not None:
        st, thresh, zout = softmax
        d.loader, d.sm_stats, d.sm_nt, d.sm_thresh, d.sm_zout = L.LOAD_SOFTMAX, st.data_ptr(), (K + 31) // 32, float(thresh), L.ptr(zout)
    if sb:
        _group(d, batch, strideA, strideW, strideC, sb)
    if plan_only:
        return int(L.load().sp3_gemm_plan(C.byref(d)))
    _gemm_launch(d, "sp3_gemm", "softmax" if softmax is not None else "plain")
    return out


def reduce_ln(partial, splits, rows, C_, *, bias=None, res=None, ldres=0, x_out=None, ldx=0,
              ln1=None, out1=None, ld1=0, ln2=None, out2=None, ld2=0, eps=1e-6, act=ACT_NONE, res2=None, ldres2=0):
    d = L.ReduceLnDesc()
    d.partial, d.split_stride, d.splits, d.rows, d.C = partial.data_ptr(), rows * C_, splits, rows, C_
    d.bias, d.res, d.ldres = L.ptr(bias), L.ptr(res), ldres or C_
    d.x_out, d.ldx = L.ptr(x_out), ldx or C_
    d.act, d.res2, d.ldres2 = act, L.ptr(res2), ldres2 or C_
    if out1 is not None:
        d.g1, d.b1, d.out1, d.ld1, d.out1_bf16 = ln1[0].data_ptr(), ln1[1].data_ptr(), out1.data_ptr(), ld1 or C_, int(out1.dtype == torch.bfloat16)
        d.out1_packed = _is_packed(out1)
    if out2 is not None:
        d.g2, d.b2, d.out2, d.ld2, d.out2_bf16 = ln2[0].data_ptr(), ln2[1].data_ptr(), out2.data_ptr(), ld2 or C_, int(out2.dtype == torch.bfloat16)
        d.out2_packed = _is_packed(out2)
    d.eps = eps
    nln = (out1 is not None) + (out2 is not None)
    _timed("reduce_ln", (splits + 8.0 * nln) * rows * C_, 4.0 * rows * C_ * (splits + 2 + nln),
           lambda: L.check(L.load().sp3_reduce_ln(C.byref(d), L.stream_ptr()), "sp3_reduce_ln"))


_TILE_PX = {None: 0, "8x8": 1, "8x16": 2, "8x16n32": 3}


def _conv_desc(Wp, xdt, odt, rdt, *, B, H, W_, Cin, Cout, stride, act, relu_in, res2_up):
    bf = torch.bfloat16
    OH, OW = (H - 1) // stride + 1, (W_ - 1) // stride + 1
    d = GemmDesc()
    d.a_bf16, d.out_bf16, d.res_bf16 = int(xdt == bf), int(odt == bf), int(rdt == bf)
    _w(d, Wp)
    d.M, d.N, d.K, d.batch = B * OH * OW, Cout, 9 * Cin, 1
    d.lda, d.ldc, d.ldr1, d.ldr2 = Cin, Cout, Cout, Cout
    d.alpha, d.act, d.relu_in = 1.0, act, int(relu_in)
    d.loader, d.epi, d.tile = L.LOAD_CONV3X3, L.EPI_PLAIN, -1
    d.conv_H, d.conv_W, d.conv_C, d.conv_OH, d.conv_OW, d.conv_stride = H, W_, Cin, OH, OW, stride
    if res2_up is not None:
        d.res2_up_H, d.res2_up_W = res2_up
    return d


def _conv_route(d, Wp, tile=-1, force_tile_kernel=False):
    free = tile < 0 and isinstance(Wp, PackedWeight)
    if (free and Wp.dtype == torch.bfloat16 and d.conv_stride == 1 and d.conv_C % 64 == 0 and d.N % 64 == 0 and d.conv_C <= 768
            and (force_tile_kernel or d.M >= 2048)):
        return "tile"
    if free:
        p = GemmDesc.from_buffer_copy(d)
        p.A, p.C = p.A or 4096, p.C or 4096
        if L.load().sp3_gemm_plan(C.byref(p)) >= 30:
            return "lean"
    return "general"


def conv3x3(x, Wp, out, *, B, H, W_, Cin, Cout, stride=1, bias=None, res1=None, res2=None, act=ACT_NONE,
            relu_in=False, tile=-1, force_tile_kernel=False, splitk_ws=None, tile_px=None, res2_up=None):
    _act(x, "x")
    rbf = [t.dtype == torch.bfloat16 for t in (res1, res2) if t is not None]
    mixed = bool(rbf) and any(rbf) != all(rbf)
    d = _conv_desc(Wp, x.dtype, out.dtype, torch.bfloat16 if any(rbf) else torch.float32, B=B, H=H, W_=W_, Cin=Cin, Cout=Cout,
                   stride=stride, act=act, relu_in=relu_in, res2_up=res2_up)
    d.A, d.C, d.bias, d.res1, d.res2 = x.data_ptr(), out.data_ptr(), L.ptr(bias), L.ptr(res1), L.ptr(res2)
    M = d.M
    route = _conv_route(d, Wp, tile, force_tile_kernel)
    if route == "tile":
        if res2_up is not None:
            raise ValueError("conv3x3: a half-resolution res2 is read by the lean small-map kernels only (B*H*W=%d)" % (B * H * W_))
        if mixed or (any(rbf) and out.dtype != torch.bfloat16):
            raise TypeError("conv3x3: residual maps must share one dtype (bf16 only next to a bf16 output)")
        _timed("conv3x3_tile", 2.0 * B * H * W_ * Cout * 9 * Cin,
               B * H * W_ * (x.element_size() * Cin + out.element_size() * Cout) + 2.0 * 9 * Cin * Cout,
               lambda: L.check(L.load().sp3_conv3x3_tile(
                   x.data_ptr(), d.a_bf16, Wp.data_ptr(), L.ptr(bias), L.ptr(res1), L.ptr(res2),
                   out.data_ptr(), d.out_bf16, d.res_bf16, _TILE_PX[tile_px], B, H, W_, Cin, Cout, int(relu_in), act,
                   L.stream_ptr()), "sp3_conv3x3_tile"))
        return out
    if mixed and tile < 0 and isinstance(Wp, PackedWeight):
        raise TypeError("conv3x3: residual maps must share one dtype")
    if route == "lean":
        _gemm_launch(d, "sp3_gemm(conv3x3)", "conv3x3")
        return out
    if res2_up is not None:
        raise ValueError("conv3x3: a half-resolution res2 is read by the lean small-map kernels only (B*H*W=%d)" % (B * H * W_))
    if any(rbf):
        raise TypeError("conv3x3: bf16 residual maps are served by the lean small-map and the LDS-tiled kernels only "
                        "(B*H*W=%d, Cin=%d, Cout=%d, stride %d)" % (B * H * W_, Cin, Cout, stride))
    S = conv_splitk(M, Cout, 9 * Cin, Wp.dtype) if (splitk_ws is not None and tile < 0 and out.dtype == torch.float32) else 1
    if S > 1 and splitk_ws.numel() < S * M * Cout:
        raise ValueError("conv3x3: splitk_ws holds %d floats, needs %d" % (splitk_ws.numel(), S * M * Cout))
    d.tile = tile
    if S > 1:
        d.C, d.bias, d.res1, d.res2 = splitk_ws.data_ptr(), None, None, None
        d.act, d.epi, d.tile, d.splitk = ACT_NONE, L.EPI_PARTIAL, 0, S
    global _held
    held, _held = _held, None
    try:
        _gemm_launch(d, "sp3_gemm(conv3x3)", "conv3x3")
    finally:
        _held = held
    if S > 1:
        reduce_ln(splitk_ws, S, M, Cout, bias=bias, res=res1, ldres=Cout, x_out=out, ldx=Cout, act=act, res2=res2, ldres2=Cout)
    return out


def conv3x3_takes_res2_up(Wp, map_dtype, B, H, W_):
    d = _conv_desc(Wp, map_dtype, map_dtype, map_dtype, B=B, H=H, W_=W_, Cin=Wp.K // 9, Cout=Wp.N, stride=1, act=ACT_NONE, relu_in=False,
                   res2_up=((H + 1) // 2, (W_ + 1) // 2))
    d.res1 = d.res2 = 4096
    return _conv_route(d, Wp) == "lean"


def conv_splitk(M, N, K, wdtype):
    tiles = ((M + 31) // 32) * ((N + 31) // 32)
    nkb = K // (64 if wdtype == torch.bfloat16 else 32)
    s = 1
    while tiles * s * 2 <= 512 and nkb // (s * 2) >= 4 and s < 8:
        s *= 2
    return s


def conv_transpose_ks(x, Wp, out, *, B, H, W_, Cin, Cout, ks, bias=None, tile=-1):
    d = GemmDesc()
    d.a_bf16 = _act(x, "x")
    d.out_bf16 = int(out.dtype == torch.bfloat16)
    _w(d, Wp)
    d.A, d.C, d.bias = x.data_ptr(), out.data_ptr(), L.ptr(bias)
    d.M, d.N, d.K, d.batch = B * H * W_, ks * ks * Cout, Cin, 1
    d.lda, d.ldc = Cin, Cout
    d.alpha = 1.0
    d.loader, d.epi, d.tile = L.LOAD_PLAIN, L.EPI_PIXSHUF, tile
    d.ps_k, d.ps_H, d.ps_W, d.ps_C = ks, H, W_, Cout
    _gemm_launch(d, "sp3_gemm(conv_transpose)", "plain")
    return out


def proj_rope_vt(A, W, bias, out_qk, ldc, vt, vt_ld, *, M, N, K, lda, rope_cols, pos, cos, sin, tokens, heads, tile=-1,
                 qkv_packed=False, ln=None, batch=1, strideA=0, strideW=0, strideC=0, sb=None):
    d = GemmDesc()
    d.a_bf16 = _act(A, "A")
    d.a_packed = _is_packed(A)
    _w(d, W)
    d.A, d.C, d.bias = A.data_ptr(), L.ptr(out_qk), L.ptr(bias)
    d.M, d.N, d.K, d.batch = M, N, K, 1
    d.lda, d.ldc = lda, ldc
    d.alpha = 1.0
    d.loader, d.epi, d.tile = L.LOAD_PLAIN, L.EPI_ROPE_VT, tile
    d.rope_cos, d.rope_sin, d.pos, d.rope_cols = cos.data_ptr(), sin.data_ptr(), pos.data_ptr(), rope_cols
    d.vt, d.vt_ld, d.tokens, d.heads = L.ptr(vt), vt_ld, tokens, heads
    d.qkv_packed = int(qkv_packed)
    _ln(d, ln)
    if out_qk is None:
        d.C = vt.data_ptr()
    if batch > 1:
        _group(d, batch, strideA, strideW, strideC, sb)
    _gemm_launch(d, "sp3_gemm(rope_vt)", "plain")


def layernorm(x, gamma, beta, eps, out, *, rows, C_, ldx=None, ldo=None, transposed=False, dual=None, group_rows=0):
    _f32(x, "x")
    ldx = C_ if ldx is None else ldx
    ldo = C_ if ldo is None else ldo
    if dual is not None:
        assert dual.dtype == torch.bfloat16 and not transposed and not _is_packed(out)
        pad = getattr(dual, "rows_pad", (group_rows + 15) // 16 * 16)
        _timed("layernorm", 8.0 * rows * C_, rows * C_ * 10.0,
               lambda: L.check(L.load().sp3_layernorm_dual(x.data_ptr(), ldx, gamma.data_ptr(), beta.data_ptr(), eps, out.data_ptr(), ldo,
                                                           dual.data_ptr(), rows, C_, group_rows or rows, pad, L.stream_ptr()),
                               "sp3_layernorm_dual"))
        return out
    if _is_packed(out):
        _timed("layernorm", 8.0 * rows * C_, rows * C_ * 6.0,
               lambda: L.check(L.load().sp3_layernorm_packed(x.data_ptr(), ldx, gamma.data_ptr(), beta.data_ptr(), eps,
                                                             out.data_ptr(), int(out.dtype == torch.bfloat16), rows, C_,
                                                             L.stream_ptr()), "sp3_layernorm_packed"))
        return out
    fn = L.load().sp3_layernorm_t if transposed else L.load().sp3_layernorm
    _timed("layernorm_t" if transposed else "layernorm", 8.0 * rows * C_, rows * C_ * (4.0 + out.element_size()),
           lambda: L.check(fn(x.data_ptr(), ldx, gamma.data_ptr(), beta.data_ptr(), eps, out.data_ptr(), ldo,
                              int(out.dtype == torch.bfloat16), rows, C_, L.stream_ptr()), "sp3_layernorm"))
    return out


def rope_2d(tokens, positions, base, fwd):
    if tokens.dim() != 4:
        raise RuntimeError("tokens must have 4 dimensions")
    if positions.dim() != 3:
        raise RuntimeError("positions must have 3 dimensions")
    if tokens.size(0) != positions.size(0):
        raise RuntimeError("batch size differs between tokens & positions")
    if tokens.size(1) != positions.size(1):
        raise RuntimeError("seq_length differs between tokens & positions")
    if positions.size(2) != 2:
# ... 173 lines not shown
    _timed("pack_bf16_conv3x3", 0.0, rows * cols * 2.0 * (bool(want) + bool(want_t)) + x.numel() * 4.0,
           lambda: L.check(L.load().sp3_pack_bf16_conv3x3(x.data_ptr(), B, H, W_, C_, stride, int(act), L.ptr(a), L.ptr(t), L.stream_ptr()), "sp3_pack_bf16_conv3x3"))
    return a, t


def gather_packed_rows(src, dst, sel, n_sel, C_):
    L.check(L.load().sp3_gather_packed_rows(src.data_ptr(), dst.data_ptr(), sel.data_ptr(), n_sel, C_, src.element_size(),
                                            L.stream_ptr()), "sp3_gather_packed_rows")


def gather_packed_cols(src, dst, sel, n_sel, n_fill, C_, cap):
    L.check(L.load().sp3_gather_packed_cols(src.data_ptr(), dst.data_ptr(), sel.data_ptr(), n_sel, n_fill, C_, cap, src.element_size(),
                                            L.stream_ptr()), "sp3_gather_packed_cols")


def prob_merge(stats, scale, rows, M, cap, dyn_n=None):
    L.check(L.load().sp3_prob_merge(stats.data_ptr(), scale.data_ptr(), rows, M, cap, L.ptr(dyn_n), L.stream_ptr()), "sp3_prob_merge")


def colsum_prob(p_packed, scale, rows, M, cap, mem_attn, dyn_n=None):
    _timed("colsum_prob", 2.0 * rows * M, 2.0 * rows * M,
           lambda: L.check(L.load().sp3_colsum_prob(p_packed.data_ptr(), scale.data_ptr(), rows, M, cap, L.ptr(dyn_n), mem_attn.data_ptr(), L.stream_ptr()),
                           "sp3_colsum_prob"))


def bank_state_set(state, M, wm):
    L.check(L.load().sp3_bank_state_set(state.data_ptr(), int(M), int(wm), L.stream_ptr()), "sp3_bank_state_set")


def cos_sim_state(k, k_raw, Tmax, P, C_, state, score, scratch):
    assert scratch.numel() >= Tmax * P and scratch.dtype == torch.float32 and state.dtype == torch.int32
    L.check(L.load().sp3_cos_sim_state(k.data_ptr(), k_raw.data_ptr(), Tmax, P, C_, state.data_ptr(), scratch.data_ptr(), score.data_ptr(),
                                       L.stream_ptr()), "sp3_cos_sim_state")


def cos_sim(k, wm, T, P, C_, score, scratch):
    assert scratch.numel() >= T * P and scratch.dtype == torch.float32
    L.check(L.load().sp3_cos_sim(k.data_ptr(), wm.data_ptr(), T, P, C_, scratch.data_ptr(), score.data_ptr(), L.stream_ptr()),
            "sp3_cos_sim")


def mem_append(count, attn, M, P):
    L.check(L.load().sp3_mem_append(count.data_ptr(), attn.data_ptr(), M, P, L.stream_ptr()), "sp3_mem_append")


def prune_select(attn, count, M, protect, top_k, sel):
    L.check(L.load().sp3_prune_select(attn.data_ptr(), count.data_ptr(), M, float(protect), top_k, sel.data_ptr(),
                                      L.stream_ptr()), "sp3_prune_select")


def gather_rows(src, dst, sel, n_sel, C_):
    L.check(L.load().sp3_gather_rows(src.data_ptr(), dst.data_ptr(), sel.data_ptr(), n_sel, C_, src.element_size(),
                                     L.stream_ptr()), "sp3_gather_rows")


def gather_cols(src, ld_src, dst, ld_dst, sel, n_sel, n_fill, C_):
    L.check(L.load().sp3_gather_cols(src.data_ptr(), ld_src, dst.data_ptr(), ld_dst, sel.data_ptr(), n_sel, n_fill, C_,
                                     src.element_size(), L.stream_ptr()), "sp3_gather_cols")


def gather_1d(src, dst, sel, n_sel):
    L.check(L.load().sp3_gather_1d(src.data_ptr(), dst.data_ptr(), sel.data_ptr(), n_sel, L.stream_ptr()), "sp3_gather_1d")


def im2col_patch(img, out, *, B, C_, H, W_, p, strides):
    _f32(img, "img")
    sb, sc, sy, sx = strides
    L.check(L.load().sp3_im2col_patch(img.data_ptr(), sb, sc, sy, sx, B, C_, H, W_, p, out.data_ptr(),
                                      int(out.dtype == torch.bfloat16), _is_packed(out), L.stream_ptr()), "sp3_im2col_patch")
    return out


def upsample2x(x, out, *, B, H, W_, C_, outH=None, outW=None):
    outH = 2 * H if outH is None else outH
    outW = 2 * W_ if outW is None else outW
    if x.dtype != out.dtype or x.dtype not in (torch.float32, torch.bfloat16):
        raise TypeError("upsample2x: fp32 or bf16 maps, input and output alike")
    fn = L.load().sp3_upsample2x_bf16 if x.dtype == torch.bfloat16 else L.load().sp3_upsample2x
    _timed("upsample2x", 8.0 * B * outH * outW * C_, float(x.element_size()) * B * C_ * (H * W_ + outH * outW),
           lambda: L.check(fn(x.data_ptr(), out.data_ptr(), B, H, W_, C_, outH, outW, L.stream_ptr()), "sp3_upsample2x"))
    return out


def head_final(feat, w, b, pixels, C_, pts, conf, raw=None):
    fn = L.load().sp3_head_final_bf16 if feat.dtype == torch.bfloat16 else L.load().sp3_head_final
    _timed("head_final", 8.0 * pixels * C_, pixels * (float(feat.element_size()) * C_ + 16.0),
           lambda: L.check(fn(feat.data_ptr(), w.data_ptr(), b.data_ptr(), pixels, C_, pts.data_ptr(),
                              conf.data_ptr(), L.ptr(raw), L.stream_ptr()), "sp3_head_final"))


def fill(t, v):
    L.check(L.load().sp3_fill_f32(t.data_ptr(), float(v), t.numel(), L.stream_ptr()), "sp3_fill_f32")


def copy2d(src, lds, dst, ldd, rows, cols):
    L.check(L.load().sp3_copy2d_f32(src.data_ptr(), lds, dst.data_ptr(), ldd, rows, cols, L.stream_ptr()), "sp3_copy2d_f32")
```

Baseline: 658.6 frames/s.

## Fuse DPT head seams: upsampled residual, 1x1-conv+upsample, patchified head output

Adds three fusions in the DPT head path. The 8x16 wide conv3x3 kernel can now read a half-resolution bf16 residual and bilinearly upsample it in the epilogue. A new kernel computes a 1x1 conv and writes its bilinear 2x upsample directly from LDS. The bf16 head_final kernel can also write the point map straight into the packed patch operand used by value encoding. Together these drop separate upsample kernels, intermediate full-resolution maps and an im2col pass, at the cost of more template variants and more complex epilogues.

Result: no change. 661.9 frames/s (median of 6 runs) (+0.5%).

```diff
diff --git a/include/spann3r_hip.h b/include/spann3r_hip.h
--- a/include/spann3r_hip.h
+++ b/include/spann3r_hip.h
@@ -181,14 +181,20 @@
 int sp3_conv3x3_tile(const void* x, int in_bf16, const void* w_packed, const float* bias, const float* res1,
                      const float* res2, void* out, int out_bf16, int res_bf16, int tile_px, int B, int H, int W,
                      int Cin, int Cout, int relu_in, int act, void* stream);
+int sp3_conv3x3_tile_up(const void* x, int in_bf16, const void* w_packed, const float* bias, const float* res1,
+                        const float* res2, void* out, int out_bf16, int res_bf16, int tile_px, int B, int H, int W,
+                        int Cin, int Cout, int relu_in, int act, int up_H, int up_W, void* stream);
+int sp3_conv3x3_tile_plan(int tile_px, int B, int H, int W, int Cin, int Cout);
 int sp3_im2col_patch(const float* img, int64_t sb, int64_t sc, int64_t sy, int64_t sx, int B, int C, int H, int W,
                      int p, void* out, int out_bf16, int out_packed, void* stream);
 int sp3_upsample2x(const float* in, float* out, int B, int H, int W, int C, int outH, int outW, void* stream);
 int sp3_upsample2x_bf16(const void* in, void* out, int B, int H, int W, int C, int outH, int outW, void* stream);
+int sp3_conv1x1_up2x(const void* x, const void* w_packed, const float* bias, void* out, int B, int H, int W, int K, int N,
+                     int outH, int outW, void* stream);
 int sp3_head_final(const float* feat, const float* w, const float* b, int64_t pixels, int C, float* pts,
                    float* conf, float* raw, void* stream);
 int sp3_head_final_bf16(const void* feat, const float* w, const float* b, int64_t pixels, int C, float* pts, float* conf,
-                        float* raw, void* stream);
+                        float* raw, void* patch_out, int p, int H, int W, void* stream);
 
 int sp3_preprocess_image(const uint8_t* src, int64_t src_row_stride, int crop_l, int crop_t, int H1, int W1,
                          const int32_t* hbounds, const int32_t* hcoef, int hksize, int W2,
diff --git a/spann3r_amd/csrc/conv.hip b/spann3r_amd/csrc/conv.hip
--- a/spann3r_amd/csrc/conv.hip
+++ b/spann3r_amd/csrc/conv.hip
@@ -16,6 +16,7 @@
   const void* x; const __bf16* w; const float* bias; const float* res1; const float* res2; void* out;
   int B, H, W, Cin, Cout, tiles_x, tiles_y, relu_in, act, out_bf16;
   int xcd_nb;
+  int up_H, up_W;
 };
 
 __device__ __forceinline__ bool conv_tile_of(const ConvArgs& a, int& t, int& nblk) {
@@ -215,7 +216,7 @@
   return HALO_BYTES > 4 * 64 * (16 * NF + 4) * 4 ? HALO_BYTES : 4 * 64 * (16 * NF + 4) * 4;
 }
 
-template <typename TIN, int NF = 4, int ABL = 0, bool WS = false>
+template <typename TIN, int NF = 4, int ABL = 0, bool WS = false, bool UP = false>
 __global__ __launch_bounds__(256, 2) void conv3x3_wide_kernel(const ConvArgs a) {
   constexpr int BN = 16 * NF, SLAB_LD = BN + 4;
   constexpr int DEPTH = NF == 2 ? 9 : 3;
@@ -379,7 +380,18 @@
       const int64_t off = (((int64_t)b * a.H + oy) * a.W + ox) * a.Cout + gn;
       if (a.out_bf16 & 2) {
         if (a.res1) { const bf16x4 q = *reinterpret_cast<const bf16x4*>(reinterpret_cast<const __bf16*>(a.res1) + off); v.x += (float)q[0]; v.y += (float)q[1]; v.z += (float)q[2]; v.w += (float)q[3]; }
-        if (a.res2) { const bf16x4 q = *reinterpret_cast<const bf16x4*>(reinterpret_cast<const __bf16*>(a.res2) + off); v.x += (float)q[0]; v.y += (float)q[1]; v.z += (float)q[2]; v.w += (float)q[3]; }
+        if constexpr (UP) {
+          const Up2xTaps up = up2x_taps(a.up_H, a.up_W, oy, ox);
+          const __bf16* src = reinterpret_cast<const __bf16*>(a.res2) + (int64_t)b * a.up_H * a.up_W * a.Cout + gn;
+          const bf16x4 u00 = *reinterpret_cast<const bf16x4*>(src + (int64_t)up.p00 * a.Cout), u01 = *reinterpret_cast<const bf16x4*>(src + (int64_t)up.p01 * a.Cout);
+          const bf16x4 u10 = *reinterpret_cast<const bf16x4*>(src + (int64_t)up.p10 * a.Cout), u11 = *reinterpret_cast<const bf16x4*>(src + (int64_t)up.p11 * a.Cout);
+          v.x += (float)(__bf16)up2x_mix(up, (float)u00[0], (float)u01[0], (float)u10[0], (float)u11[0]);
+          v.y += (float)(__bf16)up2x_mix(up, (float)u00[1], (float)u01[1], (float)u10[1], (float)u11[1]);
+          v.z += (float)(__bf16)up2x_mix(up, (float)u00[2], (float)u01[2], (float)u10[2], (float)u11[2]);
+          v.w += (float)(__bf16)up2x_mix(up, (float)u00[3], (float)u01[3], (float)u10[3], (float)u11[3]);
+        } else {
+          if (a.res2) { const bf16x4 q = *reinterpret_cast<const bf16x4*>(reinterpret_cast<const __bf16*>(a.res2) + off); v.x += (float)q[0]; v.y += (float)q[1]; v.z += (float)q[2]; v.w += (float)q[3]; }
+        }
       } else {
         if (a.res1) { const float4 q = *reinterpret_cast<const float4*>(a.res1 + off); v.x += q.x; v.y += q.y; v.z += q.z; v.w += q.w; }
         if (a.res2) { const float4 q = *reinterpret_cast<const float4*>(a.res2 + off); v.x += q.x; v.y += q.y; v.z += q.z; v.w += q.w; }
@@ -395,10 +407,10 @@
   }
 }
 
-template <typename TIN, int NF, bool WS>
+template <typename TIN, int NF, bool WS, bool UP = false>
 int launch(dim3 grid, hipStream_t st, const ConvArgs& a) {
   constexpr int lds = lds_bytes<NF>();
-  auto kern = conv3x3_wide_kernel<TIN, NF, 0, WS>;
+  auto kern = conv3x3_wide_kernel<TIN, NF, 0, WS, UP>;
   if (lds > 64 * 1024) {
     static bool raised = false;
     if (!raised) {
@@ -414,9 +426,30 @@
 
 }
 
+static int conv_tile_nf(int want, int B, int H, int W, int Cin, int Cout) {
+  const int wtx = (W + wide::TW - 1) / wide::TW, wty = (H + wide::TH - 1) / wide::TH;
+  const int64_t wgs = (int64_t)wtx * wty * B * (Cout / 64);
+  const bool can = Cin % wide::CH == 0;
+  return want == 2 ? 4 : want == 3 ? 2 : (want == 0 && can) ? (wgs >= SP3_CONV_WIDE_MIN_WGS ? 4 : wgs >= 80 ? 2 : 0) : 0;
+}
+
+extern "C" int sp3_conv3x3_tile_plan(int tile_px, int B, int H, int W, int Cin, int Cout) {
+  if (tile_px < 0 || tile_px > 3 || B <= 0 || H <= 0 || W <= 0 || Cin < 64 || Cin % 64 || Cout < 64 || Cout % 64) return -1;
+  if (tile_px >= 2 && Cin % wide::CH) return -1;
+  const int nf = conv_tile_nf(tile_px, B, H, W, Cin, Cout);
+  return nf == 4 ? 2 : nf == 2 ? 3 : 1;
+}
+
 extern "C" int sp3_conv3x3_tile(const void* x, int in_bf16, const void* w_packed, const float* bias, const float* res1,
                                 const float* res2, void* out, int out_bf16, int res_bf16, int tile_px, int B, int H, int W,
                                 int Cin, int Cout, int relu_in, int act, void* stream) {
+  return sp3_conv3x3_tile_up(x, in_bf16, w_packed, bias, res1, res2, out, out_bf16, res_bf16, tile_px, B, H, W, Cin, Cout, relu_in, act, 0, 0,
+                             stream);
+}
+
+extern "C" int sp3_conv3x3_tile_up(const void* x, int in_bf16, const void* w_packed, const float* bias, const float* res1,
+                                   const float* res2, void* out, int out_bf16, int res_bf16, int tile_px, int B, int H, int W,
+                                   int Cin, int Cout, int relu_in, int act, int up_H, int up_W, void* stream) {
   SP3_CHECK(x && w_packed && out, "sp3_conv3x3_tile: null pointer");
   SP3_CHECK(B > 0 && H > 0 && W > 0, "sp3_conv3x3_tile: bad shape");
   SP3_CHECK(Cin % 64 == 0 && Cin >= 64 && Cout % 64 == 0 && Cout >= 64, "sp3_conv3x3_tile: Cin=%d / Cout=%d must be multiples of 64", Cin, Cout);
@@ -431,23 +464,29 @@
   a.B = B; a.H = H; a.W = W; a.Cin = Cin; a.Cout = Cout;
   a.relu_in = relu_in; a.act = act; a.out_bf16 = out_bf16 | (res_bf16 << 1);
   a.xcd_nb = 0;
+  a.up_H = up_H; a.up_W = up_W;
+  const bool up = up_H != 0 || up_W != 0;
+  if (up) {
+    SP3_CHECK(up_H > 0 && up_W > 0 && res2 && in_bf16 && out_bf16 && res_bf16, "sp3_conv3x3_tile: a half-resolution res2 (%d x %d) needs res2 and bf16 map, output and residuals", up_H, up_W);
+    SP3_CHECK(H <= 2 * up_H && W <= 2 * up_W, "sp3_conv3x3_tile: a %d x %d map is no crop of the x2 of %d x %d", H, W, up_H, up_W);
+  }
   constexpr bool xcd_on = true;
   hipStream_t st = reinterpret_cast<hipStream_t>(stream);
   {
-    const int want = tile_px;
     const int wtx = (W + wide::TW - 1) / wide::TW, wty = (H + wide::TH - 1) / wide::TH;
-    const int64_t wgs = (int64_t)wtx * wty * B * (Cout / 64);
-    const bool can = Cin % wide::CH == 0;
-    SP3_CHECK(want < 2 || can, "sp3_conv3x3_tile: the 8 x 16 tile needs Cin %% 128 == 0 (Cin=%d)", Cin);
+    SP3_CHECK(tile_px < 2 || Cin % wide::CH == 0, "sp3_conv3x3_tile: the 8 x 16 tile needs Cin %% 128 == 0 (Cin=%d)", Cin);
     SP3_CHECK((int64_t)H * W * Cin * (in_bf16 ? 2 : 4) < (1ll << 31), "sp3_conv3x3_tile: one image of the map must stay below 2 GiB");
-    const int nf = want == 2 ? 4 : want == 3 ? 2 : (want == 0 && can) ? (wgs >= SP3_CONV_WIDE_MIN_WGS ? 4 : wgs >= 80 ? 2 : 0) : 0;
+    const int nf = conv_tile_nf(tile_px, B, H, W, Cin, Cout);
+    SP3_CHECK(!up || nf, "sp3_conv3x3_tile: a half-resolution res2 is read by the 8 x 16 tiles only (sp3_conv3x3_tile_plan: B=%d %d x %d Cin=%d Cout=%d)", B, H, W, Cin, Cout);
     if (nf) {
       a.tiles_x = wtx; a.tiles_y = wty;
       dim3 grid(wtx * wty * B, Cout / (16 * nf));
       if (xcd_on) { a.xcd_nb = Cout / (16 * nf); grid = dim3((unsigned)(((wtx * wty * B + 7) / 8) * 8 * a.xcd_nb), 1); }
       const bool ws = sp3_weight_streams(SP3_WF_CONV_WIDE, nf);
       int rc;
-      if (nf == 4) rc = in_bf16 ? (ws ? wide::launch<__bf16, 4, true>(grid, st, a) : wide::launch<__bf16, 4, false>(grid, st, a))
+      if (up)      rc = nf == 4 ? (ws ? wide::launch<__bf16, 4, true, true>(grid, st, a) : wide::launch<__bf16, 4, false, true>(grid, st, a))
+                                : (ws ? wide::launch<__bf16, 2, true, true>(grid, st, a) : wide::launch<__bf16, 2, false, true>(grid, st, a));
+      else if (nf == 4) rc = in_bf16 ? (ws ? wide::launch<__bf16, 4, true>(grid, st, a) : wide::launch<__bf16, 4, false>(grid, st, a))
                                 : (ws ? wide::launch<float, 4, true>(grid, st, a) : wide::launch<float, 4, false>(grid, st, a));
       else         rc = in_bf16 ? (ws ? wide::launch<__bf16, 2, true>(grid, st, a) : wide::launch<__bf16, 2, false>(grid, st, a))
                                 : (ws ? wide::launch<float, 2, true>(grid, st, a) : wide::launch<float, 2, false>(grid, st, a));
diff --git a/spann3r_amd/csrc/dpt.hip b/spann3r_amd/csrc/dpt.hip
--- a/spann3r_amd/csrc/dpt.hip
+++ b/spann3r_amd/csrc/dpt.hip
@@ -99,6 +99,98 @@
   st_out(reinterpret_cast<bf16x8*>(out + (((int64_t)b * outH + oy) * outW + ox) * C + cg * 8), o);
 }
 
+namespace c1u {
+constexpr int DH = 8, DW = 16, SH = 6, SW = 10, BN = 64, NF = BN / 16, LD = BN + 8;
+
+__global__ __launch_bounds__(256) void conv1x1_up2x_kernel(const __bf16* __restrict__ x, const __bf16* __restrict__ w,
+                                                           const float* __restrict__ bias, __bf16* __restrict__ out, int H, int W,
+                                                           int K, int N, int outH, int outW, int tiles_x) {
+  __shared__ __attribute__((aligned(16))) __bf16 tile[4 * 16 * LD];
+  const int tid = threadIdx.x, lane = tid & 63, wave = tid >> 6, g = lane >> 4, r = lane & 15;
+  const int ty = blockIdx.x / tiles_x, tx = blockIdx.x - ty * tiles_x;
+  const int n0 = blockIdx.y * BN, b = blockIdx.z;
+  const int oy0 = ty * DH, ox0 = tx * DW;
+  const Up2xTaps t0 = up2x_taps(H, W, oy0, ox0);
+  const int ys = t0.p00 / W, xs = t0.p00 - ys * W;
+
+  const int sp = 16 * wave + r;
+  int sy = ys + sp / SW, sx = xs + sp % SW;
+  sy = sy < H - 1 ? sy : H - 1;
+  sx = sx < W - 1 ? sx : W - 1;
+  const __bf16* arow = x + (((int64_t)b * H + sy) * W + sx) * K + 16 * g;
+  const int nkb = K >> 6;
+  const __bf16* wb[NF];
+#pragma unroll
+  for (int n = 0; n < NF; ++n) wb[n] = w + ((int64_t)((n0 >> 4) + n) * nkb * 128 + lane) * 8;
+  const float bv[NF] = {bias ? bias[n0 + r] : 0.f, bias ? bias[n0 + 16 + r] : 0.f, bias ? bias[n0 + 32 + r] : 0.f, bias ? bias[n0 + 48 + r] : 0.f};
+
+  struct Stage { bf16x8 a[2][2]; bf16x8 wv[2][NF][2]; };
+  auto load = [&](Stage& s, int kb0) {
+#pragma unroll
+    for (int j = 0; j < 2; ++j) {
+      int kb = kb0 + j;
+      kb = kb < nkb ? kb : nkb - 1;
+#pragma unroll
+      for (int h = 0; h < 2; ++h) {
+        s.a[j][h] = *reinterpret_cast<const bf16x8*>(arow + kb * 64 + 8 * h);
+#pragma unroll
+        for (int n = 0; n < NF; ++n) s.wv[j][n][h] = *reinterpret_cast<const bf16x8*>(wb[n] + ((int64_t)kb * 128 + h * 64) * 8);
+      }
+    }
+  };
+  f32x4 acc[NF];
+#pragma unroll
+  for (int n = 0; n < NF; ++n) acc[n] = f32x4{0.f, 0.f, 0.f, 0.f};
+  auto mma = [&](const Stage& s, int kb0) {
+#pragma unroll
+    for (int j = 0; j < 2; ++j) {
+      if (kb0 + j < nkb) {
+#pragma unroll
+        for (int n = 0; n < NF; ++n) {
+          acc[n] = __builtin_amdgcn_mfma_f32_16x16x32_bf16(s.a[j][0], s.wv[j][n][0], acc[n], 0, 0, 0);
+          acc[n] = __builtin_amdgcn_mfma_f32_16x16x32_bf16(s.a[j][1], s.wv[j][n][1], acc[n], 0, 0, 0);
+        }
+      }
+    }
+  };
+  Stage s0, s1;
+  load(s0, 0);
+  load(s1, 2);
+  for (int kb0 = 0; kb0 < nkb; kb0 += 4) {
+    mma(s0, kb0);
+    if (kb0 + 4 < nkb) load(s0, kb0 + 4);
+    mma(s1, kb0 + 2);
+    if (kb0 + 6 < nkb) load(s1, kb0 + 6);
+  }
+
+#pragma unroll
+  for (int n = 0; n < NF; ++n)
+#pragma unroll
+    for (int q = 0; q < 4; ++q) tile[(16 * wave + 4 * g + q) * LD + n * 16 + r] = (__bf16)(acc[n][q] + bv[n]);
+  __syncthreads();
+
+  for (int idx = tid; idx < DH * DW * (BN / 8); idx += 256) {
+    const int cg = idx & 7, dp = idx >> 3;
+    const int oy = oy0 + dp / DW, ox = ox0 + dp % DW;
+    if (oy >= outH || ox >= outW) continue;
+    const Up2xTaps up = up2x_taps(H, W, oy, ox);
+    const int y0 = up.p00 / W, x0 = up.p00 - y0 * W;
+    int ly0 = y0 - ys, lx0 = x0 - xs;
+    ly0 = ly0 < SH - 1 ? ly0 : SH - 1;
+    lx0 = lx0 < SW - 1 ? lx0 : SW - 1;
+    const int ly1 = (up.p10 != up.p00 && ly0 < SH - 1) ? ly0 + 1 : ly0, lx1 = (up.p01 != up.p00 && lx0 < SW - 1) ? lx0 + 1 : lx0;
+    const bf16x8 v00 = *reinterpret_cast<const bf16x8*>(tile + (ly0 * SW + lx0) * LD + cg * 8);
+    const bf16x8 v01 = *reinterpret_cast<const bf16x8*>(tile + (ly0 * SW + lx1) * LD + cg * 8);
+    const bf16x8 v10 = *reinterpret_cast<const bf16x8*>(tile + (ly1 * SW + lx0) * LD + cg * 8);
+    const bf16x8 v11 = *reinterpret_cast<const bf16x8*>(tile + (ly1 * SW + lx1) * LD + cg * 8);
+    bf16x8 o;
+#pragma unroll
+    for (int e = 0; e < 8; ++e) o[e] = (__bf16)up2x_mix(up, (float)v00[e], (float)v01[e], (float)v10[e], (float)v11[e]);
+    st_out(reinterpret_cast<bf16x8*>(out + (((int64_t)b * outH + oy) * outW + ox) * N + n0 + cg * 8), o);
+  }
+}
+}
+
 template <typename T>
 __global__ __launch_bounds__(256) void head_final_kernel(const T* __restrict__ feat, const float* __restrict__ w,
                                                          const float* __restrict__ bias, int64_t pixels, int C,
@@ -136,11 +228,13 @@
   }
 }
 
-template <int LP, int PPT>
+template <int LP, int PPT, bool PATCH>
 __global__ __launch_bounds__(256) void head_final_bf16x8_kernel(const __bf16* __restrict__ feat, const float* __restrict__ w,
                                                                 const float* __restrict__ bias, int64_t pixels, float* __restrict__ pts,
-                                                                float* __restrict__ conf, float* __restrict__ raw) {
+                                                                float* __restrict__ conf, float* __restrict__ raw,
+                                                                __bf16* __restrict__ patch_out, int p, int H, int W) {
   constexpr int C = 8 * LP, PPB = 256 / LP;
+  __shared__ __attribute__((aligned(16))) __bf16 ps[PATCH ? 3 * PPB * PPT : 8];
   const int li = threadIdx.x % LP, pl = threadIdx.x / LP;
   float wr[4][8];
 #pragma unroll
@@ -179,6 +273,25 @@
       const float sc = expm1f(d) / fmaxf(d, 1e-8f);
       pts[pix * 3 + 0] = X * sc; pts[pix * 3 + 1] = Y * sc; pts[pix * 3 + 2] = Z * sc;
       conf[pix] = 1.0f + expf(Cc);
+      if constexpr (PATCH) {
+        const int lp = q * PPB + pl;
+        ps[lp] = (__bf16)(X * sc); ps[PPB * PPT + lp] = (__bf16)(Y * sc); ps[2 * PPB * PPT + lp] = (__bf16)(Z * sc);
+      }
+    }
+  }
+  if constexpr (PATCH) {
+    __syncthreads();
+    constexpr int NCH = PPB * PPT / 8;
+    if (threadIdx.x < 3 * NCH) {
+      const int c = threadIdx.x / NCH, j = threadIdx.x - c * NCH;
+      const int64_t pix = (int64_t)blockIdx.x * PPB * PPT + 8 * j;
+      if (pix < pixels) {
+        const int hw = H * W, b = (int)(pix / hw), rem = (int)(pix - (int64_t)b * hw);
+        const int y = rem / W, x = rem - y * W;
+        const int ty = y / p, iy = y - ty * p, tx = x / p, ix = x - tx * p;
+        const int row = (b * (H / p) + ty) * (W / p) + tx, k = c * p * p + iy * p + ix;
+        *reinterpret_cast<bf16x8*>(patch_out + packed_off(row, k, 3 * p * p, true)) = *reinterpret_cast<const bf16x8*>(ps + c * PPB * PPT + 8 * j);
+      }
     }
   }
 }
@@ -224,6 +337,23 @@
   return 0;
 }
 
+extern "C" int sp3_conv1x1_up2x(const void* x, const void* w_packed, const float* bias, void* out, int B, int H, int W, int K, int N,
+                                int outH, int outW, void* stream) {
+  SP3_CHECK(x && w_packed && out && B > 0 && H > 0 && W > 0, "sp3_conv1x1_up2x: bad arguments");
+  SP3_CHECK(K >= 64 && K % 64 == 0 && N >= 64 && N % 64 == 0, "sp3_conv1x1_up2x: K=%d / N=%d must be multiples of 64", K, N);
+  SP3_CHECK(outH > 0 && outH <= 2 * H && outW > 0 && outW <= 2 * W, "sp3_conv1x1_up2x: bad crop");
+  auto al16 = [](const void* q) { return (reinterpret_cast<uintptr_t>(q) & 15) == 0; };
+  SP3_CHECK(al16(x) && al16(w_packed) && al16(out), "sp3_conv1x1_up2x: 16-byte alignment");
+  const int tiles_x = (outW + c1u::DW - 1) / c1u::DW, tiles_y = (outH + c1u::DH - 1) / c1u::DH;
+  SP3_CHECK(N / c1u::BN <= 65535 && B <= 65535 && (int64_t)tiles_x * tiles_y < (1ll << 31) && (int64_t)2 * H * 2 * W < (1ll << 31),
+            "sp3_conv1x1_up2x: grid too large");
+  hipLaunchKernelGGL(c1u::conv1x1_up2x_kernel, dim3(tiles_x * tiles_y, N / c1u::BN, B), dim3(256), 0, ST(stream),
+                     reinterpret_cast<const __bf16*>(x), reinterpret_cast<const __bf16*>(w_packed), bias,
+                     reinterpret_cast<__bf16*>(out), H, W, K, N, outH, outW, tiles_x);
+  SP3_LAUNCH_CHECK("sp3_conv1x1_up2x");
+  return 0;
+}
+
 extern "C" int sp3_head_final(const float* feat, const float* w, const float* b, int64_t pixels, int C, float* pts, float* conf,
                               float* raw, void* stream) {
   SP3_CHECK(feat && w && b && pts && conf && pixels > 0 && C > 0 && C % 32 == 0, "sp3_head_final: bad arguments");
@@ -235,12 +365,24 @@
 }
 
 extern "C" int sp3_head_final_bf16(const void* feat, const float* w, const float* b, int64_t pixels, int C, float* pts, float* conf,
-                                   float* raw, void* stream) {
+                                   float* raw, void* patch_out, int p, int H, int W, void* stream) {
   SP3_CHECK(feat && w && b && pts && conf && pixels > 0 && C > 0 && C % 32 == 0, "sp3_head_final_bf16: bad arguments");
+  if (patch_out) {
+    SP3_CHECK(C == 128, "sp3_head_final_bf16: the patch operand is written by the 128-channel kernel only (C=%d)", C);
+    SP3_CHECK(p > 0 && p % 8 == 0 && H > 0 && W > 0 && H % p == 0 && W % p == 0 && pixels % ((int64_t)H * W) == 0 && pixels < (1ll << 31),
+              "sp3_head_final_bf16: patch operand of %lld pixels as %d x %d images in %d x %d patches (a multiple of 8)", (long long)pixels, H, W, p, p);
+    SP3_CHECK((reinterpret_cast<uintptr_t>(feat) & 15) == 0 && (reinterpret_cast<uintptr_t>(w) & 15) == 0 && (!raw || (reinterpret_cast<uintptr_t>(raw) & 15) == 0),
+              "sp3_head_final_bf16: 16-byte alignment");
+    constexpr int LP = 16, PPT = 4, PPB = 256 / LP;
+    hipLaunchKernelGGL((head_final_bf16x8_kernel<LP, PPT, true>), dim3((unsigned)((pixels + PPB * PPT - 1) / (PPB * PPT))), dim3(256), 0, ST(stream),
+                       reinterpret_cast<const __bf16*>(feat), w, b, pixels, pts, conf, raw, reinterpret_cast<__bf16*>(patch_out), p, H, W);
+    SP3_LAUNCH_CHECK("sp3_head_final_bf16");
+    return 0;
+  }
   if (C == 128 && (reinterpret_cast<uintptr_t>(feat) & 15) == 0 && (reinterpret_cast<uintptr_t>(w) & 15) == 0 && (!raw || (reinterpret_cast<uintptr_t>(raw) & 15) == 0)) {
     constexpr int LP = 16, PPT = 4, PPB = 256 / LP;
-    hipLaunchKernelGGL((head_final_bf16x8_kernel<LP, PPT>), dim3((unsigned)((pixels + PPB * PPT - 1) / (PPB * PPT))), dim3(256), 0, ST(stream),
-                       reinterpret_cast<const __bf16*>(feat), w, b, pixels, pts, conf, raw);
+    hipLaunchKernelGGL((head_final_bf16x8_kernel<LP, PPT, false>), dim3((unsigned)((pixels + PPB * PPT - 1) / (PPB * PPT))), dim3(256), 0, ST(stream),
+                       reinterpret_cast<const __bf16*>(feat), w, b, pixels, pts, conf, raw, static_cast<__bf16*>(nullptr), 0, 0, 0);
     SP3_LAUNCH_CHECK("sp3_head_final_bf16");
     return 0;
   }
diff --git a/spann3r_amd/engine.py b/spann3r_amd/engine.py
--- a/spann3r_amd/engine.py
+++ b/spann3r_amd/engine.py
@@ -586,35 +586,39 @@
                     splitk_ws=self._conv_ws(tag[:1]))
         return t
 
-    def _rcu(self, x, pre, B, H, W_, out, extra_res=None, tag="", c1_done=False, extra_up=None):
+    def _rcu(self, x, pre, B, H, W_, out, extra_res=None, tag="", c1_done=False, extra_up=None, up_px=None):
         w, F = self.w, self.cfg.dpt_feat
         t = self.ws("rcu_tmp" + tag, (B * H * W_, F), self.mdt)
         if not c1_done:
             self._rcu_c1(x, pre, B, H, W_, tag)
         ops.conv3x3(t, w[pre + "c2.w"], out, B=B, H=H, W_=W_, Cin=F, Cout=F, bias=w[pre + "c2.b"], res1=x, res2=extra_res,
-                    splitk_ws=self._conv_ws(tag[:1]), res2_up=extra_up)
+                    splitk_ws=self._conv_ws(tag[:1]), res2_up=extra_up, tile_px=up_px)
         return out
 
-    def _fusion(self, pre, B, H, W_, x0, x1, tag, crop=None, c1_done=False, x0_up=None, fold_up=False):
+    def _fusion(self, pre, B, H, W_, x0, x1, tag, crop=None, c1_done=False, x0_up=None, fold_up=False, x0_px=None, fuse_up=False):
         w, F = self.w, self.cfg.dpt_feat
         M = B * H * W_
         cur = x0
         if x1 is not None:
             s = self.ws("fus_sum_" + tag, (M, F), self.mdt)
-            self._rcu(x1, pre + "u1", B, H, W_, s, extra_res=x0, tag=tag, c1_done=c1_done, extra_up=x0_up)
+            self._rcu(x1, pre + "u1", B, H, W_, s, extra_res=x0, tag=tag, c1_done=c1_done, extra_up=x0_up, up_px=x0_px)
             cur = s
         r = self.ws("fus_rcu2_" + tag, (M, F), self.mdt)
         self._rcu(cur, pre + "u2", B, H, W_, r, tag=tag, c1_done=c1_done and x1 is None)
+        OH, OW = (2 * H, 2 * W_) if crop is None else crop
+        if fuse_up and not fold_up and ops.conv1x1_up2x_matches(r, w[pre + "out.w"], B=B, H=H, W_=W_, K=F, N=F, bias=w[pre + "out.b"]):
+            up = self.ws("fus_up_" + tag, (B * OH * OW, F), self.mdt)
+            ops.conv1x1_up2x(r, w[pre + "out.w"], up, B=B, H=H, W_=W_, K=F, N=F, bias=w[pre + "out.b"], outH=OH, outW=OW)
+            return up, OH, OW
         oc = self.ws("fus_oc_" + tag, (M, F), self.mdt)
         ops.gemm(r, w[pre + "out.w"], oc, M=M, N=F, K=F, lda=F, ldc=F, bias=w[pre + "out.b"])
-        OH, OW = (2 * H, 2 * W_) if crop is None else crop
         if fold_up:
             return oc, OH, OW
         up = self.ws("fus_up_" + tag, (B * OH * OW, F), self.mdt)
         ops.upsample2x(oc, up, B=B, H=H, W_=W_, C_=F, outH=OH, outW=OW)
         return up, OH, OW
 
-    def dpt_head(self, dec, B, nh, nw, num, want_raw=False):
+    def dpt_head(self, dec, B, nh, nw, num, want_raw=False, patch_out=None):
         self.activate()
         cfg, w = self.cfg, self.w
         F, Lc = cfg.dpt_feat, cfg.dpt_last
@@ -671,13 +675,13 @@
             pp3c()
             for i in range(4):
                 layer_rn(i)
-        path, up, Hc, Wc = rn[3], None, h3, w3
+        path, up, up_px, Hc, Wc = rn[3], None, None, h3, w3
         for j in range(4):
             Hn, Wn = geo[3 - j]
-            fold = lv and j < 3 and ops.conv3x3_takes_res2_up(w[refs[j + 1][0] + "u1c2.w"], mdt, B, *geo[2 - j])
+            fold = lv and j < 3 and ops.conv3x3_takes_res2_up(w[refs[j + 1][0] + "u1c2.w"], mdt, B, *geo[2 - j], tiled=ops.head_seam("a"))
             nxt, OH_, OW_ = self._fusion(refs[j][0], B, Hn, Wn, path, rn[3 - j] if j else None, refs[j][1], crop=(nh, nw) if j == 0 else None,
-                                         c1_done=lv, x0_up=up, fold_up=fold)
-            path, up = nxt, ((Hn, Wn) if fold else None)
+                                         c1_done=lv, x0_up=up, fold_up=bool(fold), x0_px=up_px, fuse_up=lv and ops.head_seam("b"))
+            path, up, up_px = nxt, ((Hn, Wn) if fold else None), (fold if isinstance(fold, str) else None)
         p1, H1, W1 = path, OH_, OW_
         a = self.ws("dpt%d_h0" % num, (B * H1 * W1, Lc), mdt)
         ops.conv3x3(p1, w[pre + "h0.w"], a, B=B, H=H1, W_=W1, Cin=F, Cout=Lc, bias=w[pre + "h0.b"])
@@ -689,8 +693,19 @@
         pts = self.ws("dpt_pts%d" % num, (B, OH, OW, 3))
         conf = self.ws("dpt_conf%d" % num, (B, OH, OW))
         raw = self.ws("dpt_raw%d" % num, (B, OH, OW, 4)) if want_raw else None
-        ops.head_final(c, w[pre + "h4.w"], w[pre + "h4.b"], B * OH * OW, Lc, pts, conf, raw)
+        patch = None
+        if patch_out is not None:
+            assert (OH, OW) == (nh * cfg.patch, nw * cfg.patch)
+            patch = (patch_out, cfg.patch, OH, OW)
+        ops.head_final(c, w[pre + "h4.w"], w[pre + "h4.b"], B * OH * OW, Lc, pts, conf, raw, patch=patch)
         return pts, conf, raw
+
+    def value_patch_operand(self, B, nh, nw):
+        cfg = self.cfg
+        if not ops.head_seam("c") or cfg.use_feat or not ops.head_final_takes_patch(self.mdt, cfg.dpt_last, cfg.patch):
+            return None
+        col = self.wsp("im2col_val", B * nh * nw, 3 * cfg.patch * cfg.patch)
+        return col if col.dtype == torch.bfloat16 else None
 
     def encode_cur_value_feat(self, tok, out, res, pos32=None):
         self.activate()
@@ -715,7 +730,7 @@
                  ln=ops.LnFold(stA, Cv, w["value_out.s"], 1e-6))
         return out
 
-    def encode_cur_value(self, pts3d, out, res):
+    def encode_cur_value(self, pts3d, out, res, col=None):
         self.activate()
         cfg, w = self.cfg, self.w
         B, H, W_, _ = pts3d.shape
@@ -724,9 +739,12 @@
         P = nh * nw
         R = B * P
         _, pos32, zero_pos = self.positions(B, nh, nw)
-        col = self.wsp("im2col_val", R, 3 * p * p)
-        sb, sy, sx, sc = pts3d.stride()
-        ops.im2col_patch(pts3d, col, B=B, C_=3, H=H, W_=W_, p=p, strides=(sb, sc, sy, sx))
+        if col is None:
+            col = self.wsp("im2col_val", R, 3 * p * p)
+            sb, sy, sx, sc = pts3d.stride()
+            ops.im2col_patch(pts3d, col, B=B, C_=3, H=H, W_=W_, p=p, strides=(sb, sc, sy, sx))
+        else:
+            assert (col.M, col.K) == (R, 3 * p * p)
         x, xp, st = self._vit(col, R, B, P, "pospatch", "val", cfg.val_depth, pos32 if cfg.mem_pos_enc else zero_pos, tag="_val")
         ops.gemm(xp, w["value_out.w"], out, M=R, N=E, K=E, lda=E, ldc=E, bias=w["value_out.b"], res1=res, ldr1=E,
                  ln=ops.LnFold(st, E, w["value_out.s"], 1e-6))
diff --git a/spann3r_amd/lib.py b/spann3r_amd/lib.py
--- a/spann3r_amd/lib.py
+++ b/spann3r_amd/lib.py
@@ -179,12 +179,17 @@
                          C.c_int, C.c_void_p, C.c_int, C.c_int, C.c_void_p],
     "sp3_conv3x3_tile": [C.c_void_p, C.c_int, C.c_void_p, C.c_void_p, C.c_void_p, C.c_void_p, C.c_void_p, C.c_int, C.c_int, C.c_int,
                          C.c_int, C.c_int, C.c_int, C.c_int, C.c_int, C.c_int, C.c_int, C.c_void_p],
+    "sp3_conv3x3_tile_up": [C.c_void_p, C.c_int, C.c_void_p, C.c_void_p, C.c_void_p, C.c_void_p, C.c_void_p, C.c_int, C.c_int, C.c_int,
+                            C.c_int, C.c_int, C.c_int, C.c_int, C.c_int, C.c_int, C.c_int, C.c_int, C.c_int, C.c_void_p],
+    "sp3_conv3x3_tile_plan": [C.c_int, C.c_int, C.c_int, C.c_int, C.c_int, C.c_int],
+    "sp3_conv1x1_up2x": [C.c_void_p, C.c_void_p, C.c_void_p, C.c_void_p, C.c_int, C.c_int, C.c_int, C.c_int, C.c_int, C.c_int, C.c_int,
+                         C.c_void_p],
     "sp3_upsample2x": [C.c_void_p, C.c_void_p, C.c_int, C.c_int, C.c_int, C.c_int, C.c_int, C.c_int, C.c_void_p],
     "sp3_head_final": [C.c_void_p, C.c_void_p, C.c_void_p, C.c_int64, C.c_int, C.c_void_p, C.c_void_p, C.c_void_p,
                        C.c_void_p],
     "sp3_upsample2x_bf16": [C.c_void_p, C.c_void_p, C.c_int, C.c_int, C.c_int, C.c_int, C.c_int, C.c_int, C.c_void_p],
     "sp3_head_final_bf16": [C.c_void_p, C.c_void_p, C.c_void_p, C.c_int64, C.c_int, C.c_void_p, C.c_void_p, C.c_void_p,
-                            C.c_void_p],
+                            C.c_void_p, C.c_int, C.c_int, C.c_int, C.c_void_p],
     "sp3_fill_f32": [C.c_void_p, C.c_float, C.c_int64, C.c_void_p],
     "sp3_cast_f32_to_bf16": [C.c_void_p, C.c_void_p, C.c_int64, C.c_void_p],
     "sp3_copy2d_f32": [C.c_void_p, C.c_int64, C.c_void_p, C.c_int64, C.c_int, C.c_int, C.c_void_p],
diff --git a/spann3r_amd/model.py b/spann3r_amd/model.py
--- a/spann3r_amd/model.py
+++ b/spann3r_amd/model.py
@@ -739,12 +739,13 @@
             st[2].wait_stream(main)
             with torch.cuda.stream(st[2]):
                 pts2, conf2, _ = eng.dpt_head(dec2, B, self.hh, self.hw, 2)
-        pts1, conf1, _ = eng.dpt_head(dec1, B, self.hh, self.hw, 1)
+        col = None if self.swap else eng.value_patch_operand(B, self.hh, self.hw)
+        pts1, conf1, _ = eng.dpt_head(dec1, B, self.hh, self.hw, 1, patch_out=col)
         if eng.cfg.use_feat:
             eng.encode_cur_value_feat(dec1[-1], self.v, self.k1,
                                       pos32=eng.positions(B, self.nh, self.nw)[1] if eng.cfg.mem_pos_enc else None)
         else:
-            eng.encode_cur_value(pts1.swapaxes(1, 2) if self.swap else pts1, self.v, self.k1)
+            eng.encode_cur_value(pts1.swapaxes(1, 2) if self.swap else pts1, self.v, self.k1, col=col)
         mem.stage_write(self.k1, self.v)
         if not self.defer2:
             main.wait_stream(st[2])
diff --git a/spann3r_amd/ops.py b/spann3r_amd/ops.py
--- a/spann3r_amd/ops.py
+++ b/spann3r_amd/ops.py
@@ -102,6 +102,13 @@
 LEAN = _os.environ.get("SP3_LEAN_GEMM", "1")[:1] != "0"
 
 HEAD_LEVELS = _os.environ.get("SP3_HEAD_LEVELS", "1")[:1] != "0"
+HEAD_SEAMS = {"0": False, "1": True}.get(_os.environ.get("SP3_HEAD_SEAMS", "1"), _os.environ.get("SP3_HEAD_SEAMS", "1"))
+
+
+def head_seam(piece):
+    return piece in HEAD_SEAMS if isinstance(HEAD_SEAMS, str) else bool(HEAD_SEAMS)
+
+
 _held = None
 
 
@@ -428,6 +435,11 @@
 
 
 _TILE_PX = {None: 0, "8x8": 1, "8x16": 2, "8x16n32": 3}
+_TILE_PX_NAMES = {v: k for k, v in _TILE_PX.items() if k}
+
+
+def conv3x3_tile_plan(B, H, W_, Cin, Cout, tile_px=None):
+    return _TILE_PX_NAMES.get(L.load().sp3_conv3x3_tile_plan(_TILE_PX[tile_px], B, H, W_, Cin, Cout))
 
 
 def _conv_desc(Wp, xdt, odt, rdt, *, B, H, W_, Cin, Cout, stride, act, relu_in, res2_up):
@@ -470,15 +482,17 @@
     M = d.M
     route = _conv_route(d, Wp, tile, force_tile_kernel)
     if route == "tile":
-        if res2_up is not None:
-            raise ValueError("conv3x3: a half-resolution res2 is read by the lean small-map kernels only (B*H*W=%d)" % (B * H * W_))
+        if res2_up is not None and not (tile_px in ("8x16", "8x16n32") and d.a_bf16 and d.out_bf16 and d.res_bf16 and res2 is not None):
+            raise ValueError("conv3x3: a half-resolution res2 is read by the lean small-map kernels and by the 8 x 16 tiles named in "
+                             "tile_px on bf16 maps only (B*H*W=%d)" % (B * H * W_))
         if mixed or (any(rbf) and out.dtype != torch.bfloat16):
             raise TypeError("conv3x3: residual maps must share one dtype (bf16 only next to a bf16 output)")
+        uh, uw = res2_up if res2_up is not None else (0, 0)
         _timed("conv3x3_tile", 2.0 * B * H * W_ * Cout * 9 * Cin,
                B * H * W_ * (x.element_size() * Cin + out.element_size() * Cout) + 2.0 * 9 * Cin * Cout,
-               lambda: L.check(L.load().sp3_conv3x3_tile(
+               lambda: L.check(L.load().sp3_conv3x3_tile_up(
                    x.data_ptr(), d.a_bf16, Wp.data_ptr(), L.ptr(bias), L.ptr(res1), L.ptr(res2),
-                   out.data_ptr(), d.out_bf16, d.res_bf16, _TILE_PX[tile_px], B, H, W_, Cin, Cout, int(relu_in), act,
+                   out.data_ptr(), d.out_bf16, d.res_bf16, _TILE_PX[tile_px], B, H, W_, Cin, Cout, int(relu_in), act, uh, uw,
                    L.stream_ptr()), "sp3_conv3x3_tile"))
         return out
     if mixed and tile < 0 and isinstance(Wp, PackedWeight):
@@ -509,11 +523,15 @@
     return out
 
 
-def conv3x3_takes_res2_up(Wp, map_dtype, B, H, W_):
+def conv3x3_takes_res2_up(Wp, map_dtype, B, H, W_, tiled=False):
     d = _conv_desc(Wp, map_dtype, map_dtype, map_dtype, B=B, H=H, W_=W_, Cin=Wp.K // 9, Cout=Wp.N, stride=1, act=ACT_NONE, relu_in=False,
                    res2_up=((H + 1) // 2, (W_ + 1) // 2))
     d.res1 = d.res2 = 4096
-    return _conv_route(d, Wp) == "lean"
+    route = _conv_route(d, Wp)
+    if tiled and route == "tile" and map_dtype == torch.bfloat16:
+        px = conv3x3_tile_plan(B, H, W_, Wp.K // 9, Wp.N)
+        return px if px in ("8x16", "8x16n32") else False
+    return route == "lean"
 
 
 def conv_splitk(M, N, K, wdtype):
@@ -853,11 +871,51 @@
     return out
 
 
-def head_final(feat, w, b, pixels, C_, pts, conf, raw=None):
-    fn = L.load().sp3_head_final_bf16 if feat.dtype == torch.bfloat16 else L.load().sp3_head_final
+_GEMM_TILES_ONE_ACC = (1, 2)
+
+
+def conv1x1_up2x_matches(x, Wp, *, B, H, W_, K, N, bias=None):
+    if not (x.dtype == torch.bfloat16 and isinstance(Wp, PackedWeight) and Wp.dtype == torch.bfloat16 and not Wp.halves
+            and K % 64 == 0 and N % 64 == 0 and (Wp.N, Wp.K) == (N, K)):
+        return False
+    M = B * H * W_
+    return gemm(x, Wp, x, M=M, N=N, K=K, lda=K, ldc=N, bias=bias, plan_only=True) in _GEMM_TILES_ONE_ACC
+
+
+def conv1x1_up2x(x, Wp, out, *, B, H, W_, K, N, bias=None, outH=None, outW=None):
+    outH = 2 * H if outH is None else outH
+    outW = 2 * W_ if outW is None else outW
+    if not (x.dtype == out.dtype == torch.bfloat16 and isinstance(Wp, PackedWeight) and Wp.dtype == torch.bfloat16 and not Wp.halves
+            and (Wp.N, Wp.K) == (N, K)):
+        raise TypeError("conv1x1_up2x: bf16 maps and a bf16 PackedWeight [%d, %d]" % (N, K))
+    _timed("conv1x1_up2x", 2.0 * B * H * W_ * N * K + 8.0 * B * outH * outW * N, 2.0 * (B * H * W_ * K + N * K + B * outH * outW * N),
+           lambda: L.check(L.load().sp3_conv1x1_up2x(x.data_ptr(), Wp.data_ptr(), L.ptr(bias), out.data_ptr(), B, H, W_, K, N, outH, outW,
+                                                     L.stream_ptr()), "sp3_conv1x1_up2x"))
+    return out
+
+
+def head_final_takes_patch(map_dtype, C_, p=16):
+    return map_dtype == torch.bfloat16 and C_ == 128 and p % 8 == 0
+
+
+def head_final(feat, w, b, pixels, C_, pts, conf, raw=None, patch=None):
+    if patch is not None:
+        col, p, H, W_ = patch
+        if not (head_final_takes_patch(feat.dtype, C_, p) and isinstance(col, PackedAct) and col.dtype == torch.bfloat16
+                and pixels % (H * W_) == 0 and col.M == pixels // (p * p) and col.K == 3 * p * p):
+            raise ValueError("head_final: no patch operand [%d, %d] from %d pixels of a %s map with %d channels"
+                             % (getattr(col, "M", -1), getattr(col, "K", -1), pixels, feat.dtype, C_))
+        _timed("head_final", 8.0 * pixels * C_, pixels * (float(feat.element_size()) * C_ + 22.0),
+               lambda: L.check(L.load().sp3_head_final_bf16(feat.data_ptr(), w.data_ptr(), b.data_ptr(), pixels, C_, pts.data_ptr(),
+                                                            conf.data_ptr(), L.ptr(raw), col.data_ptr(), p, H, W_, L.stream_ptr()),
+                               "sp3_head_final"))
+        return
+    bf = feat.dtype == torch.bfloat16
+    fn = L.load().sp3_head_final_bf16 if bf else L.load().sp3_head_final
+    tail = (None, 0, 0, 0, L.stream_ptr()) if bf else (L.stream_ptr(),)
     _timed("head_final", 8.0 * pixels * C_, pixels * (float(feat.element_size()) * C_ + 16.0),
            lambda: L.check(fn(feat.data_ptr(), w.data_ptr(), b.data_ptr(), pixels, C_, pts.data_ptr(),
-                              conf.data_ptr(), L.ptr(raw), L.stream_ptr()), "sp3_head_final"))
+                              conf.data_ptr(), L.ptr(raw), *tail), "sp3_head_final"))
 
 
 def fill(t, v):
```
